# rubiruchi/ofdm_uhd

Hardware: AMD Instinct MI355X
Metric: OFDM symbols/sec (TX+loopback RX) @ N_fft=512; packet CRC pass rate (higher is better)
Workload: dtype f32; 1 GPU; N_fft=512, occ=200, QPSK, CP=128, synthetic AWGN channel (BASELINE configs[1]); payload_bytes=1026, symbols_per_packet=22, streams=1, iq_buffers=1, parallelism=independent streams, 1 per GPU

## Files before the change

ofdm_uhd_amd/csrc/engine_rx.inc:

```

template <typename T>
static int dev_excl_scan(ofdm_handle* h, const T* d_in, uint64_t n, T* d_out, T* d_total) {
  const uint64_t nb = (n + SCAN_BLOCK - 1) / SCAN_BLOCK;
  HIPCHK(h, h->rx.partial.ensure(sizeof(T) * std::max<uint64_t>(nb, 1)));
  T* part = h->rx.partial.as<T>();
  if (n == 0) {
    if (d_total) HIPCHK(h, hipMemsetAsync(d_total, 0, sizeof(T), h->stream));
    return OFDM_OK;
  }
  hipLaunchKernelGGL(HIP_KERNEL_NAME(k_scan_partials<T>), dim3((unsigned)nb), dim3(256), 0, h->stream, d_in, n, part);
  hipLaunchKernelGGL(HIP_KERNEL_NAME(k_scan_top<T>), dim3(1), dim3(256), 0, h->stream, part, nb, d_total);
  hipLaunchKernelGGL(HIP_KERNEL_NAME(k_scan_final<T>), dim3((unsigned)nb), dim3(256), 0, h->stream, d_in, n, part, d_out);
  HIPCHK(h, hipGetLastError());
  return OFDM_OK;
}

template <int N, bool TWL, bool TAPS, bool CSI = false>
static int launch_demod_t(ofdm_handle* h, const DemodParams& q, size_t shmem) {
  constexpr int T = N / 8, FPW = demod_fpw(N);
  if (shmem > 64 * 1024)
    HIPCHK(h, hipFuncSetAttribute(reinterpret_cast<const void*>(&k_rx_demod<N, TWL, TAPS, CSI>),
                                  hipFuncAttributeMaxDynamicSharedMemorySize, (int)shmem));
  hipLaunchKernelGGL(HIP_KERNEL_NAME(k_rx_demod<N, TWL, TAPS, CSI>), dim3((q.nframes + FPW - 1) / FPW), dim3(T * FPW), shmem,
                     h->stream, q);
  HIPCHK(h, hipGetLastError());
  return OFDM_OK;
}
template <int N, bool TWL>
static int launch_demod_v(ofdm_handle* h, const DemodParams& q, size_t shmem) {
  if (q.csi_eq) return launch_demod_t<N, TWL, true, true>(h, q, shmem);
  const bool instr = q.tap_mode != 0 || q.tap_sampler || q.tap_fft || q.tap_acq || q.tap_sink || q.tap_demapped || q.qual;
  return instr ? launch_demod_t<N, TWL, true>(h, q, shmem) : launch_demod_t<N, TWL, false>(h, q, shmem);
}

template <int N>
static int launch_demod(ofdm_handle* h, const DemodParams& q0) {
  DemodParams q = q0;
  constexpr int T = N / 8, WAVES = demod_fpw(N) * ((T + WAVE - 1) / WAVE);
  const bool grid = q.grid != nullptr;
  const bool csi = q.csi_eq != nullptr;
  auto bytes = [&](bool twl, bool sm) {
    return (size_t)demod_lds_bytes(N, twl, sm, q.occ, q.arity, q.nmap, q.nbits, q.shift, grid, csi);
  };
  constexpr int CU_WAVES = 4 * demod_waves_per_simd(N);
  auto wgs = [&](size_t b) { return std::max<size_t>(1, std::min<size_t>(std::max(1, CU_WAVES / WAVES), CU_LDS_BYTES / b)); };
  constexpr bool base_twl = !fft_onebuf(N);
  const size_t w0 = wgs(bytes(base_twl, false));
  bool twl = base_twl;
  if constexpr (fft_onebuf(N)) twl = wgs(bytes(true, false)) == w0 && bytes(true, false) <= CU_LDS_BYTES;
  q.smap_lds = (wgs(bytes(twl, true)) == w0 && bytes(twl, true) <= CU_LDS_BYTES) ? 1 : 0;
  if (const char* e = getenv("OFDM_DEMOD_LDS")) {
    const int v = atoi(e);
    if constexpr (fft_onebuf(N)) twl = (v & 1) != 0;
    q.smap_lds = (v >> 1) & 1;
  }
  const size_t shmem = bytes(twl, q.smap_lds != 0);
  if (shmem > CU_LDS_BYTES) FAIL(h, OFDM_E_INVAL, "configuration needs more than 160 KiB of LDS in k_rx_demod");
  if constexpr (fft_onebuf(N)) {
    return twl ? launch_demod_v<N, true>(h, q, shmem) : launch_demod_v<N, false>(h, q, shmem);
  } else {
    return launch_demod_v<N, true>(h, q, shmem);
  }
}

static int run_demod(ofdm_handle* h, const DemodParams& q) {
  switch (h->N) {
    case 64: return launch_demod<64>(h, q);
    case 128: return launch_demod<128>(h, q);
    case 256: return launch_demod<256>(h, q);
    case 512: return launch_demod<512>(h, q);
    case 1024: return launch_demod<1024>(h, q);
    case 2048: return launch_demod<2048>(h, q);
    default: return launch_demod<4096>(h, q);
  }
}

enum { CT_CAND = 0, CT_OVERFLOW = 1, CT_NLO = 2, CT_NHI = 3, CT_CHAIN = 4, CT_NPEAKS = 5, CT_NSYM = 6, CT_KEYTOT = 7,
       CT_DEFR = 8 , CT_RAWTOT = 13, CT_PIECES = 14, CT_STASH = 15, CT_RECS = 16, CT_COUNT = 17 };

static int sync_params(ofdm_handle* h, uint64_t nsamples, bool cap_full, SyncParams* out) {
  RxState& rx = h->rx;
  const int N = h->N, CP = h->CP, T = SYNC_TILE;
  const uint64_t ntiles = (nsamples + T - 1) / T;
  const int tiles_per_seg = 32 * ((N + CP + T - 1) / T);
  const uint64_t egrid = std::min<uint64_t>(ntiles, 256ull * 8ull), egrid_small = std::min<uint64_t>(ntiles, 256ull * 16ull);
  const uint64_t cand_cap = (cap_full ? nsamples + nsamples / 8 : nsamples / 16) + (egrid + 16) * SYNC_CHUNK_C + egrid_small * 2048ull;
  const uint64_t piece_cap = (cap_full ? nsamples / 2 + 1 : nsamples / 128) + (egrid + egrid_small + 16) * SYNC_CHUNK_P;
  HIPCHK(h, rx.y.ensure(nsamples * sizeof(c32)));
  HIPCHK(h, rx.tile_B.ensure(ntiles * sizeof(double)));
  HIPCHK(h, rx.tile_np.ensure(ntiles * sizeof(uint32_t)));
  HIPCHK(h, rx.tile_pieces.ensure(piece_cap * sizeof(SyncPiece)));
  HIPCHK(h, rx.tile_first.ensure(ntiles * sizeof(uint64_t)));
  HIPCHK(h, rx.avg_in.ensure(ntiles * sizeof(double)));
  HIPCHK(h, rx.cand_u.ensure(cand_cap * sizeof(float)));
  HIPCHK(h, rx.cand_P.ensure(cand_cap * sizeof(c32)));
  HIPCHK(h, rx.counters.ensure(CT_COUNT * sizeof(uint64_t)));
  HIPCHK(h, rx.counts.ensure(ntiles * sizeof(uint32_t)));
  HIPCHK(h, rx.offsets.ensure(ntiles * sizeof(uint32_t)));
  HIPCHK(h, rx.recs.ensure(ntiles * sizeof(SyncRec)));
  float *d_metric = nullptr, *d_presel = nullptr;
  if (h->tap_mask & (1u << OFDM_TAP_RX_METRIC)) {
    HIPCHK(h, rx.metric.ensure(nsamples * sizeof(float)));
    d_metric = rx.metric.as<float>();
  }
  if (h->tap_mask & (1u << OFDM_TAP_RX_PRESEL)) {
    HIPCHK(h, rx.presel.ensure(nsamples * sizeof(float)));
    d_presel = rx.presel.as<float>();
  }
  uint64_t* ctr = rx.counters.as<uint64_t>();
  SyncParams sp;
  memset(&sp, 0, sizeof(sp));
  sp.N = N;
  sp.D = N / 2;
  sp.CP = CP;
  sp.HY = (N + 7) / 8 * 8;
  sp.HM = CP;
  sp.R = sync_ring_samples(sp.HY);
  sp.tiles_per_seg = tiles_per_seg;
  sp.nsamples = nsamples;
  sp.ntiles = ntiles;
  sp.tapcp = (float)(1.0 / (double)CP);
  sp.cand_thr = -fmaxf(h->cfg.peak_rise, h->cfg.peak_fall);
  sp.alpha = h->cfg.peak_alpha;
  sp.decay = (double)(1.0f - h->cfg.peak_alpha);
  sp.y = rx.y.as<c32>();
  sp.metric_tap = d_metric;
  sp.presel_tap = d_presel;
  sp.dpow = h->d_synctab.as<double>();
  sp.ipow = sp.dpow + (SYNC_TILE + 1);
  sp.wtab = reinterpret_cast<const float*>(sp.ipow + (SYNC_TILE + 1));
  sp.tile_B = rx.tile_B.as<double>();
  sp.tile_npieces = rx.tile_np.as<uint32_t>();
  sp.tile_first = rx.tile_first.as<uint64_t>();
  sp.pieces = rx.tile_pieces.as<SyncPiece>();
  sp.piece_cap = piece_cap;
  sp.piece_count = reinterpret_cast<unsigned long long*>(ctr + CT_PIECES);
  sp.cand_u = rx.cand_u.as<float>();
  sp.cand_P = rx.cand_P.as<c32>();
  sp.cand_cap = cand_cap;
  sp.cand_count = reinterpret_cast<unsigned long long*>(ctr + CT_CAND);
  sp.overflow = reinterpret_cast<unsigned int*>(ctr + CT_OVERFLOW);
  sp.recs = rx.recs.as<SyncRec>();
  sp.rec_count = reinterpret_cast<unsigned long long*>(ctr + CT_RECS);
  sp.exact_small = sync_exact_small(CP, N / 2);
  if (const char* es = getenv("OFDM_EXACT_SMALL")) sp.exact_small = std::max(0, std::min(atoi(es), (int)SYNC_TILE));
#ifdef SYNC_DIAG
  if (const char* ab = getenv("OFDM_ABLATE")) sp.ablate = atoi(ab);
#endif
  if (sp.HM > T) FAIL(h, OFDM_E_INVAL, "cyclic prefix longer than a k_sync tile");
  *out = sp;
  return OFDM_OK;
}

static uint64_t sync_nseg(const SyncParams& sp) { return (sp.ntiles + (uint64_t)sp.tiles_per_seg - 1) / (uint64_t)sp.tiles_per_seg; }

#ifdef SYNC_STAMPS
static DevBuf g_stamp_buf;
static int stamps_prepare(ofdm_handle* h, SyncParams& sp, uint64_t nseg) {
  HIPCHK(h, g_stamp_buf.ensure(nseg * 16 * sizeof(unsigned long long)));
  HIPCHK(h, hipMemsetAsync(g_stamp_buf.p, 0, nseg * 16 * sizeof(unsigned long long), h->stream));
  sp.stamps = g_stamp_buf.as<unsigned long long>();
  return OFDM_OK;
}
static int sync_stamps_report(ofdm_handle* h, const unsigned long long* d_stamps, uint64_t nseg, int tiles_per_seg) {
  HIPCHK(h, hipStreamSynchronize(h->stream));
  std::vector<unsigned long long> st(nseg * 16);
  HIPCHK(h, hipMemcpy(st.data(), d_stamps, st.size() * 8, hipMemcpyDeviceToHost));
  double sum[16] = {0};
  for (uint64_t i = 0; i < nseg; i++)
    for (int k = 0; k < 16; k++) sum[k] += (double)st[i * 16 + k];
  const char* nm[16] = {"-", "y tile -> ring / filter", "B2 wait", "terms", "scan3 (B3)", "M + B4", "mavg + B5", "summary", "filter: block A", "filter: block B", "filter: taps + windows in", "-", "-", "-", "-", "-"};
  double tot = 0;
  for (int k = 0; k < 16; k++) tot += sum[k];
  fprintf(stderr, "[k_sync stamps] %llu workgroups, s_memtime ticks per workgroup-tile (wave 0):\n", (unsigned long long)nseg);
  for (int k = 0; k < 11; k++)
    fprintf(stderr, "  %-26s %10.0f  %5.1f%%\n", nm[k], sum[k] / (double)nseg / (double)(tiles_per_seg + 1), 100.0 * sum[k] / tot);
  return OFDM_OK;
}
#endif

static bool front_fused(const ofdm_handle* h) {
  if (h->cfg.sync_mode != OFDM_SYNC_PN) return false;
  const char* e = getenv("OFDM_FRONT");
  if (!e || atoi(e) == 0) return false;
  const int F = h->filtF, B = F - (int)h->cfg.ntaps + 1;
  if (F > 512) return false;
  const int HY = (h->N + 7) / 8 * 8, C = (B + 7) / 8 * 8;
  if (HY + C > SYNC_TILE || h->CP > SYNC_TILE) return false;
  return front_lds_layout(sync_ring_samples(HY), h->CP, B, F).total <= CU_LDS_BYTES / 3;
}

static int launch_sync(ofdm_handle* h, SyncParams& sp) {
  RxState& rx = h->rx;
  const int T = SYNC_TILE;
  const uint64_t nseg = sync_nseg(sp);
  HIPCHK(h, hipMemsetAsync(rx.counters.p, 0, CT_COUNT * sizeof(uint64_t), h->stream));
#ifdef SYNC_STAMPS
  if (int rs = stamps_prepare(h, sp, nseg)) return rs;
#endif
  const size_t sync_shmem = sync_lds_layout(sp.R, sp.HM).total;
  if (sync_shmem > CU_LDS_BYTES) FAIL(h, OFDM_E_INVAL, "configuration needs more than 160 KiB of LDS in k_sync");
  {
    ProfScope span(h->prof, OFDM_K_SYNC, h->stream);
    int wg = (int)std::min<size_t>(SYNC_MAX_WG, CU_LDS_BYTES / sync_shmem);
    if (const char* w = getenv("OFDM_SYNC_W")) wg = std::min(wg, atoi(w));
    bool fixed_layout = sp.R - (int)T <= (int)T;
    if (const char* e = getenv("OFDM_SYNC_STATIC")) fixed_layout = fixed_layout && atoi(e) != 0;
    const void* fn = fixed_layout ? (wg >= 6   ? reinterpret_cast<const void*>(&k_sync<6, true>)
                                     : wg == 5 ? reinterpret_cast<const void*>(&k_sync<5, true>)
                                     : wg == 4 ? reinterpret_cast<const void*>(&k_sync<4, true>)
                                     : wg == 3 ? reinterpret_cast<const void*>(&k_sync<3, true>)
                                               : reinterpret_cast<const void*>(&k_sync<2, true>))
                                  : (wg >= 4   ? reinterpret_cast<const void*>(&k_sync<4, false>)
                                     : wg == 3 ? reinterpret_cast<const void*>(&k_sync<3, false>)
                                               : reinterpret_cast<const void*>(&k_sync<2, false>));
    HIPCHK(h, hipFuncSetAttribute(fn, hipFuncAttributeMaxDynamicSharedMemorySize, (int)sync_shmem));
    FilterParams nofp;
    memset(&nofp, 0, sizeof(nofp));
    void* args[] = {&sp, &nofp};
    HIPCHK(h, hipLaunchKernel(fn, dim3((unsigned)nseg), dim3(SYNC_THREADS), args, sync_shmem, h->stream));
  }
  HIPCHK(h, hipGetLastError());
  return OFDM_OK;
}

static void rx_note_input(ofdm_handle* h, const ofdm_c32* iq, uint64_t nsamples) {
  std::swap(h->ev_rx_in, h->ev_rx_in_old);
  h->rx_in_old_pending = h->rx_in_pending;
  h->rx_in_lo[1] = h->rx_in_lo[0];
  h->rx_in_hi[1] = h->rx_in_hi[0];
  h->rx_in_lo[0] = (uintptr_t)iq;
  h->rx_in_hi[0] = (uintptr_t)iq + nsamples * rx_ss(h);
}

static int launch_front(ofdm_handle* h, FilterParams& fp, uint64_t nsamples) {
  const int F = h->filtF;
  SyncParams sp;
  int rcs = sync_params(h, nsamples, false, &sp);
  if (rcs != OFDM_OK) return rcs;
  HIPCHK(h, hipMemsetAsync(h->rx.counters.p, 0, CT_COUNT * sizeof(uint64_t), h->stream));
  const size_t shm = front_lds_layout(sp.R, sp.HM, fp.B, F).total;
  const uint64_t nseg = sync_nseg(sp);
  const void* fn = F == 64    ? reinterpret_cast<const void*>(&k_sync<3, true, 64>)
                   : F == 128 ? reinterpret_cast<const void*>(&k_sync<3, true, 128>)
                   : F == 256 ? reinterpret_cast<const void*>(&k_sync<3, true, 256>)
                              : reinterpret_cast<const void*>(&k_sync<3, true, 512>);
  HIPCHK(h, hipFuncSetAttribute(fn, hipFuncAttributeMaxDynamicSharedMemorySize, (int)shm));
#ifdef SYNC_STAMPS
  if (int rs = stamps_prepare(h, sp, nseg)) return rs;
#endif
  void* args[] = {&sp, &fp};
  {
    ProfScope span(h->prof, OFDM_K_FRONT, h->stream);
    HIPCHK(h, hipLaunchKernel(fn, dim3((unsigned)nseg), dim3(SYNC_THREADS), args, shm, h->stream));
  }
  HIPCHK(h, hipGetLastError());
#ifdef SYNC_STAMPS
  if (int rs = sync_stamps_report(h, sp.stamps, nseg, sp.tiles_per_seg)) return rs;
#endif
  h->rx.front_done = true;
  return OFDM_OK;
}

template <typename XT>
static int launch_filter_t(ofdm_handle* h, FilterParams& fp, uint64_t nsamples) {
  const int F = h->filtF;
  const uint64_t bpr = 256 / (F / 8);
  const uint64_t nblk = (nsamples + (uint64_t)fp.goff + (uint64_t)fp.B - 1) / (uint64_t)fp.B;
  fp.nrounds = (nblk + bpr - 1) / bpr;
  const size_t fsh = (size_t)256 * 9 * sizeof(c32);
  const unsigned fgrid = (unsigned)std::min<uint64_t>(fp.nrounds, 256ull * 8ull * 4ull);
  {
    ProfScope span(h->prof, OFDM_K_FILTER, h->stream);
    switch (F) {
      case 64: hipLaunchKernelGGL(HIP_KERNEL_NAME(k_chan_filter<64, XT>), dim3(fgrid), dim3(256), fsh, h->stream, fp); break;
      case 128: hipLaunchKernelGGL(HIP_KERNEL_NAME(k_chan_filter<128, XT>), dim3(fgrid), dim3(256), fsh, h->stream, fp); break;
      case 256: hipLaunchKernelGGL(HIP_KERNEL_NAME(k_chan_filter<256, XT>), dim3(fgrid), dim3(256), fsh, h->stream, fp); break;
      case 512: hipLaunchKernelGGL(HIP_KERNEL_NAME(k_chan_filter<512, XT>), dim3(fgrid), dim3(256), fsh, h->stream, fp); break;
      case 1024: hipLaunchKernelGGL(HIP_KERNEL_NAME(k_chan_filter<1024, XT>), dim3(fgrid), dim3(256), fsh, h->stream, fp); break;
      default: FAIL(h, OFDM_E_INVAL, "unsupported channel filter transform length");
    }
  }
  HIPCHK(h, hipGetLastError());
  return OFDM_OK;
}

static int launch_filter(ofdm_handle* h, FilterParams& fp, uint64_t nsamples) {
  return h->rx_fmt == OFDM_IQ_SC16 ? launch_filter_t<sc16>(h, fp, nsamples) : launch_filter_t<c32>(h, fp, nsamples);
}

static int rx_submit_impl(ofdm_handle* h, const ofdm_c32* iq, uint64_t nsamples, const c32** d_x_out) {
  RxState& rx = h->rx;
  HIPCHK(h, hipSetDevice(h->cfg.device_id));
  if (h->tx_pending && h->txs != h->stream) HIPCHK(h, hipStreamWaitEvent(h->stream, h->ev_tx_done, 0));
  h->tx_pending = false;
  const c32* d_x = reinterpret_cast<const c32*>(iq);
  if (h->rx_fmt == OFDM_IQ_SC16) {
    if ((uintptr_t)iq & 3u) FAIL(h, OFDM_E_INVAL, "ofdm_sc16 buffers must be 4-byte aligned");
    if (front_fused(h)) FAIL(h, OFDM_E_INVAL, "the fused front end (OFDM_FRONT=1) takes float32 samples only");
  }
  if (!h->dev_ptrs) {
    HIPCHK(h, rx.x_stage.ensure(nsamples * rx_ss(h)));
    HIPCHK(h, hipMemcpyAsync(rx.x_stage.p, iq, nsamples * rx_ss(h), hipMemcpyHostToDevice, h->stream));
    d_x = rx.x_stage.as<c32>();
  }
  *d_x_out = d_x;
  rx.in_event_at_end = true;
  if (h->cfg.sync_mode != OFDM_SYNC_PN) return OFDM_OK;
  HIPCHK(h, rx.y.ensure(nsamples * sizeof(c32)));
  FilterParams fp;
  memset(&fp, 0, sizeof(fp));
  fp.B = h->filtF - (int)h->cfg.ntaps + 1;
  fp.ntm1 = (int)h->cfg.ntaps - 1;
  fp.goff = (int)(rx.origin % (uint64_t)fp.B);
  fp.nsamples = nsamples;
  fp.x = d_x;
  fp.y = rx.y.as<c32>();
  fp.Hf = h->d_Hf.as<c32>();
  fp.twF = h->d_twF.as<c32>();
  fp.xscale = h->rx_scale;
  rx.front_done = false;
  if (int rc = front_fused(h) ? launch_front(h, fp, nsamples) : launch_filter(h, fp, nsamples)) return rc;
  if (!h->sense.rx_on) {
    rx_note_input(h, iq, nsamples);
    HIPCHK(h, hipEventRecord(h->ev_rx_in, h->stream));
    h->rx_in_pending = true;
    rx.in_event_at_end = false;
  }
  return OFDM_OK;
}

extern "C" int ofdm_rx_submit(ofdm_handle* h, const ofdm_c32* iq, uint64_t nsamples) {
  if (!h) return OFDM_E_INVAL;
  if (nsamples && !iq) FAIL(h, OFDM_E_INVAL, "null argument");
  RxState& rx = h->rx;
  rx.sub_valid = false;
  if (nsamples == 0) return OFDM_OK;
  const c32* d_x = nullptr;
  int rc = rx_submit_impl(h, iq, nsamples, &d_x);
  if (rc != OFDM_OK) return rc;
  rx.sub_valid = true;
  rx.sub_iq = iq;
  rx.sub_n = nsamples;
  rx.sub_dx = d_x;
  rx.sub_hold = rx.in_event_at_end;
  return OFDM_OK;
}

struct RxCall {
  ofdm_handle* h;
  const ofdm_c32* iq;
  uint64_t nsamples;
  uint8_t* payload_out;
  uint64_t payload_cap;
  uint64_t* payload_off;
  uint32_t* payload_len;
  uint8_t* crc_ok;
  int max_pkts;
  int* npkt;
  ofdm_stats* stats;
  const c32* d_x = nullptr;
  bool fixed = false;
  bool done = false;
  bool dyn = false;
  uint64_t npeaks = 0, nforced = 0;
  uint64_t n_lo = 0, nframes = 0, nsym = 0, npk = 0, nbytes = 0, rawtot = 0;
  uint64_t npk_ub = 0;
  DynFrames dynf;
  DemodParams dq;
  DeframeParams fq;
  CsiRows csi_fr = {nullptr, nullptr, nullptr, nullptr};
  uint8_t* d_pay = nullptr;
};

static uint64_t* rx_ctr(ofdm_handle* h) { return h->rx.counters.as<uint64_t>(); }

static int rx_read_counts(RxCall& c) {
  ofdm_handle* h = c.h;
  RxState& rx = h->rx;
  uint64_t hc[CT_COUNT];
  HIPCHK(h, hipMemcpyAsync(hc, rx.counters.p, sizeof(hc), hipMemcpyDeviceToHost, h->stream));
  HIPCHK(h, hipStreamSynchronize(h->stream));
  c.n_lo = hc[CT_NLO] & 0xFFFFFFFFull;
  c.nframes = c.npeaks - c.n_lo - (hc[CT_NHI] & 0xFFFFFFFFull);
  c.nsym = hc[CT_NSYM];
  c.npk = hc[CT_KEYTOT] >> 40;
  c.nbytes = hc[CT_KEYTOT] & ((1ull << 40) - 1);
  c.rawtot = hc[CT_RAWTOT];
  rx.nframes = c.nframes;
  rx.j0 = c.n_lo;
  rx.nsym_total = c.nsym;
  if (c.stats) {
    c.stats->frames = c.nframes;
    c.stats->symbols = c.nsym;
    c.stats->headers_ok = hc[CT_DEFR + 0];
    c.stats->chained_frames = hc[CT_DEFR + 3];
    c.stats->overflow = hc[CT_OVERFLOW] & 0xFFFFFFFFull;
  }
  return OFDM_OK;
}

static int rx_check_capacity(RxCall& c) {
  if (c.npk <= (uint64_t)c.max_pkts && c.nbytes <= c.payload_cap) return OFDM_OK;
  *c.npkt = (int)std::min<uint64_t>(c.npk, 0x7FFFFFFF);
  FAIL(c.h, OFDM_E_CAPACITY, "payload_out / max_pkts too small for the packets found");
}

static hipError_t launch_sync_exact(const void* fn, unsigned grid, size_t shmem, SyncParams sp, hipStream_t s) {
  void* args[] = {&sp};
  return hipLaunchKernel(fn, dim3(grid), dim3(SYNC_THREADS), args, shmem, s);
}

static int rx_sync_exact(RxCall& c, SyncParams& sp, bool cap_full) {
  ofdm_handle* h = c.h;
  if (cap_full) {
    int rcs = sync_params(h, c.nsamples, true, &sp);
    if (rcs != OFDM_OK) return rcs;
    uint64_t* ctr = rx_ctr(h);
    HIPCHK(h, hipMemsetAsync(ctr + CT_CAND, 0, 2 * sizeof(uint64_t), h->stream));
    HIPCHK(h, hipMemsetAsync(ctr + CT_NPEAKS, 0, sizeof(uint64_t), h->stream));
    HIPCHK(h, hipMemsetAsync(ctr + CT_PIECES, 0, 2 * sizeof(uint64_t), h->stream));
  }
  const unsigned egrid = (unsigned)std::min<uint64_t>(sp.ntiles, 256ull * 8ull);
  const unsigned egrid_small = (unsigned)std::min<uint64_t>(sp.ntiles, 256ull * 16ull);
  {
    ProfScope span(h->prof, OFDM_K_EXACT, h->stream);
    const size_t esh = exact_lds_layout(sp.CP, SYNC_TILE).total, esh_small = exact_lds_layout(sp.CP, sp.exact_small).total;
    const void* fbig = sp.D >= 2048 ? reinterpret_cast<const void*>(&k_sync_exact<SYNC_THREADS, true>)
                                    : reinterpret_cast<const void*>(&k_sync_exact<SYNC_THREADS, false>);
    if (esh > 64 * 1024) HIPCHK(h, hipFuncSetAttribute(fbig, hipFuncAttributeMaxDynamicSharedMemorySize, (int)esh));
    if (sp.exact_small > 0)
      hipLaunchKernelGGL(HIP_KERNEL_NAME(k_sync_exact<WAVE, false>), dim3(egrid_small), dim3(WAVE), esh_small, h->stream, sp);
    HIPCHK(h, launch_sync_exact(fbig, egrid, esh, sp, h->stream));
    if (sp.metric_tap) {
      SyncParams tp = sp;
      tp.tap_only = 1;
      HIPCHK(h, launch_sync_exact(fbig, egrid, esh, tp, h->stream));
    }
  }
  HIPCHK(h, hipGetLastError());
#ifdef SYNC_STAMPS
  if (!h->rx.front_done)
    if (int rs = sync_stamps_report(h, sp.stamps, sync_nseg(sp), sp.tiles_per_seg)) return rs;
#endif
  return OFDM_OK;
}

static int rx_sense_fork(RxCall& c) {
  ofdm_handle* h = c.h;
  SenseState& ss = h->sense;
  HIPCHK(h, hipEventRecord(ss.ev_in, h->stream));
  HIPCHK(h, hipStreamWaitEvent(ss.side, ss.ev_in, 0));
  int src = sense_enqueue(h, &ss.rx_cfg, c.d_x, c.nsamples, ss.side);
  if (src != OFDM_OK) return src;
  HIPCHK(h, hipEventRecord(ss.ev_out, ss.side));
  return OFDM_OK;
}

static PeakParams make_peak_params(ofdm_handle* h, const SyncParams& sp) {
  RxState& rx = h->rx;
  PeakParams pp;
  memset(&pp, 0, sizeof(pp));
  pp.ntiles = sp.ntiles;
  pp.nsamples = sp.nsamples;
  pp.rise = h->cfg.peak_rise;
  pp.fall = h->cfg.peak_fall;
  pp.alpha = h->cfg.peak_alpha;
  pp.dpow = sp.dpow;
  pp.tile_npieces = rx.tile_np.as<uint32_t>();
  pp.tile_first = rx.tile_first.as<uint64_t>();
  pp.pieces = rx.tile_pieces.as<SyncPiece>();
  pp.avg_in = rx.avg_in.as<double>();
  pp.cand_u = rx.cand_u.as<float>();
  pp.cand_P = rx.cand_P.as<c32>();
  pp.counts = rx.counts.as<uint32_t>();
  pp.offsets = rx.offsets.as<uint32_t>();
  pp.stash_peaks = rx.stash_peaks.as<uint64_t>();
  pp.stash_P = rx.stash_P.as<c32>();
  pp.stash_overflow = reinterpret_cast<unsigned int*>(rx_ctr(h) + CT_STASH);
  if (h->tap_mask & (1u << OFDM_TAP_RX_RUN_AVG)) pp.run_rows = rx.run_rows.as<double>();
  return pp;
}

static int rx_flags_pn(RxCall& c, const SyncParams& sp, uint64_t* overflow) {
  ofdm_handle* h = c.h;
  RxState& rx = h->rx;
  const uint64_t ntiles = sp.ntiles;
  const unsigned grid = (unsigned)((ntiles + 255) / 256);
  uint64_t* ctr = rx_ctr(h);
  const uint64_t run_cap = (h->tap_mask & (1u << OFDM_TAP_RX_RUN_AVG)) ? sp.piece_cap : 0;
  HIPCHK(h, rx.stash_peaks.ensure(ntiles * PEAK_STASH * sizeof(uint64_t)));
  HIPCHK(h, rx.stash_P.ensure(ntiles * PEAK_STASH * sizeof(c32)));
  if (run_cap) HIPCHK(h, rx.run_rows.ensure(run_cap * 2 * sizeof(double)));
  PeakParams pp = make_peak_params(h, sp);
  hipLaunchKernelGGL(k_avg_carry, dim3(grid), dim3(256), 0, h->stream, rx.tile_B.as<double>(), ntiles, c.nsamples, sp.dpow,
                     rx.avg_in.as<double>());
  if (run_cap) HIPCHK(h, hipMemsetAsync(rx.run_rows.p, 0xFF, run_cap * 2 * sizeof(double), h->stream));
  hipLaunchKernelGGL(HIP_KERNEL_NAME(k_peak<false>), dim3(grid), dim3(256), 0, h->stream, pp);
  HIPCHK(h, hipGetLastError());
  int rc = dev_excl_scan<uint32_t>(h, rx.counts.as<uint32_t>(), ntiles, rx.offsets.as<uint32_t>(),
                                   reinterpret_cast<uint32_t*>(ctr + CT_NPEAKS));
  if (rc) return rc;
  uint64_t hc[CT_COUNT];
  HIPCHK(h, hipMemcpyAsync(hc, ctr, sizeof(hc), hipMemcpyDeviceToHost, h->stream));
  HIPCHK(h, hipStreamSynchronize(h->stream));
  if ((*overflow = hc[CT_OVERFLOW] & 0xFFFFFFFFull)) return OFDM_OK;
  rx.run_slots = std::min<uint64_t>(hc[CT_PIECES], run_cap);
  const uint64_t npeaks = hc[CT_NPEAKS] & 0xFFFFFFFFull;
  c.npeaks = rx.npeaks = npeaks;
  if (c.stats) c.stats->peaks = npeaks;
  if (npeaks == 0 && !(rx.nco_ref_on && !rx.hist_flags.empty())) {
    c.done = true;
    return OFDM_OK;
  }
  HIPCHK(h, rx.peaks.ensure(std::max<uint64_t>(npeaks, 1) * sizeof(uint64_t)));
  HIPCHK(h, rx.peak_P.ensure(std::max<uint64_t>(npeaks, 1) * sizeof(c32)));
  pp.peaks = rx.peaks.as<uint64_t>();
  pp.peak_P = rx.peak_P.as<c32>();
  if (npeaks > 0) {
    if (hc[CT_STASH] & 0xFFFFFFFFull)
      hipLaunchKernelGGL(HIP_KERNEL_NAME(k_peak<true>), dim3(grid), dim3(256), 0, h->stream, pp);
    else
      hipLaunchKernelGGL(k_peak_compact, dim3(grid), dim3(256), 0, h->stream, pp);
    HIPCHK(h, hipGetLastError());
  }
  return OFDM_OK;
}

__global__ void __launch_bounds__(256) k_fixed_flags(uint64_t npeaks, uint64_t first, uint64_t period, uint64_t* __restrict__ peaks,
                                                      c32* __restrict__ peak_P) {
  const uint64_t k = (uint64_t)blockIdx.x * blockDim.x + threadIdx.x;
  if (k >= npeaks) return;
  peaks[k] = first + k * period;
  peak_P[k] = mk(0.f, 0.f);
}

static int rx_fixed_count(RxCall& c) {
  ofdm_handle* h = c.h;
  RxState& rx = h->rx;
  const uint64_t L = (uint64_t)h->L;
  c.npeaks = rx.npeaks = c.nsamples >= L ? (c.nsamples - L) / ((uint64_t)h->cfg.fixed_nsymbols * L) + 1 : 0;
  if (c.stats) c.stats->peaks = c.npeaks;
  HIPCHK(h, rx.counters.ensure(CT_COUNT * sizeof(uint64_t)));
  HIPCHK(h, hipMemsetAsync(rx.counters.p, 0, CT_COUNT * sizeof(uint64_t), h->stream));
  if (c.npeaks == 0) {
    HIPCHK(h, hipStreamSynchronize(h->stream));
    c.done = true;
  }
  return OFDM_OK;
}

static int rx_flags_fixed(RxCall& c) {
  ofdm_handle* h = c.h;
  RxState& rx = h->rx;
  HIPCHK(h, rx.peaks.ensure(c.npeaks * sizeof(uint64_t)));
  HIPCHK(h, rx.peak_P.ensure(c.npeaks * sizeof(c32)));
  hipLaunchKernelGGL(k_fixed_flags, dim3((unsigned)((c.npeaks + 255) / 256)), dim3(256), 0, h->stream, c.npeaks, (uint64_t)h->L - 1,
                     (uint64_t)h->cfg.fixed_nsymbols * (uint64_t)h->L, rx.peaks.as<uint64_t>(), rx.peak_P.as<c32>());
  HIPCHK(h, hipGetLastError());
  return OFDM_OK;
}

static int rx_splice(RxCall& c) {
  ofdm_handle* h = c.h;
  RxState& rx = h->rx;
  if (!rx.nco_ref_on) return OFDM_OK;
  const uint64_t npeaks = c.npeaks;
  std::vector<uint64_t> hp(npeaks);
  if (npeaks) HIPCHK(h, hipMemcpyAsync(hp.data(), rx.peaks.p, npeaks * sizeof(uint64_t), hipMemcpyDeviceToHost, h->stream));
  HIPCHK(h, hipStreamSynchronize(h->stream));
  uint64_t kdrop = 0;
  while (kdrop < npeaks && (int64_t)hp[kdrop] <= rx.nco_trust_after) kdrop++;
  const uint64_t m = rx.hist_flags.size(), np2 = m + npeaks - kdrop;
  c.done = np2 == 0;
  if (!c.done) {
    HIPCHK(h, rx.peaks2.ensure(np2 * sizeof(uint64_t)));
    HIPCHK(h, rx.peak_P2.ensure(np2 * sizeof(c32)));
    HIPCHK(h, rx.fstep.ensure(std::max<uint64_t>(m, 1) * sizeof(double)));
    if (m) {
      HIPCHK(h, hipMemcpyAsync(rx.peaks2.p, rx.hist_flags.data(), m * sizeof(uint64_t), hipMemcpyHostToDevice, h->stream));
      HIPCHK(h, hipMemsetAsync(rx.peak_P2.p, 0, m * sizeof(c32), h->stream));
      HIPCHK(h, hipMemcpyAsync(rx.fstep.p, rx.hist_steps.data(), m * sizeof(double), hipMemcpyHostToDevice, h->stream));
    }
    if (npeaks > kdrop) {
      HIPCHK(h, hipMemcpyAsync(rx.peaks2.as<uint64_t>() + m, rx.peaks.as<uint64_t>() + kdrop, (npeaks - kdrop) * sizeof(uint64_t),
                               hipMemcpyDeviceToDevice, h->stream));
      HIPCHK(h, hipMemcpyAsync(rx.peak_P2.as<c32>() + m, rx.peak_P.as<c32>() + kdrop, (npeaks - kdrop) * sizeof(c32),
                               hipMemcpyDeviceToDevice, h->stream));
    }
    HIPCHK(h, hipStreamSynchronize(h->stream));
    std::swap(rx.peaks, rx.peaks2);
    std::swap(rx.peak_P, rx.peak_P2);
    c.nforced = m;
  }
  c.npeaks = rx.npeaks = np2;
  if (c.stats) c.stats->peaks = np2;
  return OFDM_OK;
}

static FramesParams make_frames_params(const RxCall& c) {
  ofdm_handle* h = c.h;
  RxState& rx = h->rx;
  uint64_t* ctr = rx_ctr(h);
  FramesParams fp;
  memset(&fp, 0, sizeof(fp));
  fp.npeaks = c.npeaks;
  fp.nsamples = c.nsamples;
  fp.N = h->N;
  fp.L = h->L;
  fp.timeout = h->cfg.sampler_timeout;
  fp.sens = (float)(-2.0 / (double)h->N);
  fp.peaks = rx.peaks.as<uint64_t>();
  fp.peak_P = rx.peak_P.as<c32>();
  fp.angle = rx.angle.as<float>();
  fp.step = rx.step.as<double>();
  fp.inc = rx.inc.as<uint64_t>();
  fp.K = rx.K.as<uint32_t>();
  fp.nsym = rx.nsym.as<uint64_t>();
  fp.n_lo = reinterpret_cast<unsigned int*>(ctr + CT_NLO);
  fp.n_hi = reinterpret_cast<unsigned int*>(ctr + CT_NHI);
  fp.nforced = c.nforced;
  fp.forced_step = rx.fstep.as<double>();
  fp.fixed_on = c.fixed ? 1 : 0;
  fp.fixed_angle = h->cfg.fixed_freq_offset;
  return fp;
}

static int rx_frames(RxCall& c) {
  ofdm_handle* h = c.h;
  RxState& rx = h->rx;
  const uint64_t npeaks = c.npeaks;
  const unsigned grid = (unsigned)((npeaks + 255) / 256);
  HIPCHK(h, rx.angle.ensure(npeaks * sizeof(float)));
  HIPCHK(h, rx.step.ensure(npeaks * sizeof(double)));
  HIPCHK(h, rx.inc.ensure(npeaks * sizeof(uint64_t)));
  HIPCHK(h, rx.inc_acc.ensure(npeaks * sizeof(uint64_t)));
  HIPCHK(h, rx.Phi_u.ensure(npeaks * sizeof(uint64_t)));
  HIPCHK(h, rx.Phi.ensure(npeaks * sizeof(double)));
  HIPCHK(h, rx.K.ensure(npeaks * sizeof(uint32_t)));
  HIPCHK(h, rx.nsym.ensure(npeaks * sizeof(uint64_t)));
  HIPCHK(h, rx.sym_base.ensure(npeaks * sizeof(uint64_t)));
  const FramesParams fp = make_frames_params(c);
  const uint64_t ref_u = rx.nco_ref_on ? rx.nco_ref_u : 0ull;
  c.dq.ref_on = (rx.nco_ref_on || (c.fixed && h->cfg.fixed_freq_offset != 0.0f)) ? 1 : 0;
  c.dq.ref_peak = rx.nco_ref_on ? rx.nco_ref_peak : 0;
  c.dq.ref_phi = nco_radians(ref_u);
  c.dq.ref_step = rx.nco_ref_on ? rx.nco_ref_step : (double)(fp.sens * h->cfg.fixed_freq_offset);
  hipLaunchKernelGGL(k_frames, dim3(grid), dim3(256), 0, h->stream, fp);
  HIPCHK(h, hipGetLastError());
  int rc = dev_excl_scan<uint64_t>(h, rx.inc.as<uint64_t>(), npeaks, rx.inc_acc.as<uint64_t>(), (uint64_t*)nullptr);
  if (rc) return rc;
  hipLaunchKernelGGL(k_nco_phase, dim3(grid), dim3(256), 0, h->stream, rx.peaks.as<uint64_t>(), rx.inc_acc.as<uint64_t>(), npeaks,
                     c.dq.ref_on, c.dq.ref_peak, ref_u, c.dq.ref_step, rx.Phi_u.as<uint64_t>(), rx.Phi.as<double>());
  HIPCHK(h, hipGetLastError());
  return dev_excl_scan<uint64_t>(h, rx.nsym.as<uint64_t>(), npeaks, rx.sym_base.as<uint64_t>(), rx_ctr(h) + CT_NSYM);
}

static int rx_timing(RxCall& c) {
  ofdm_handle* h = c.h;
  SyncParams sp;
  uint64_t overflow = 0;
  int rc = c.fixed ? rx_fixed_count(c) : sync_params(h, c.nsamples, false, &sp);
  if (rc || c.done) return rc;
  if (!c.fixed && !h->rx.front_done && (rc = launch_sync(h, sp))) return rc;
  for (int attempt = 0; attempt < 2; attempt++) {
    if (!c.fixed && (rc = rx_sync_exact(c, sp, attempt == 1))) return rc;
    if (!c.fixed && attempt == 0 && h->sense.rx_on && (rc = rx_sense_fork(c))) return rc;
    ProfScope span(h->prof, OFDM_K_PEAK, h->stream);
    if ((rc = c.fixed ? rx_flags_fixed(c) : rx_flags_pn(c, sp, &overflow))) return rc;
    if (overflow) continue;
    if (c.done) {
      span.end();
      HIPCHK(h, hipStreamSynchronize(h->stream));
      return OFDM_OK;
    }
    if ((rc = rx_splice(c)) || c.done) return rc;
    return rx_frames(c);
  }
  if (c.stats) c.stats->overflow = overflow;
  FAIL(h, OFDM_E_OVERFLOW, "candidate / piece buffer exhausted");
}

static size_t csi_bytes(uint64_t rows, uint64_t stride) { return rows * stride * (sizeof(c32) + 3 * sizeof(float)); }
static CsiRows csi_carve(const DevBuf& b, uint64_t rows, uint64_t stride) {
  const uint64_t cell = rows * stride;
  CsiRows r;
  r.eq = b.as<c32>();
  r.pre = reinterpret_cast<float*>(r.eq + cell);
  r.err = r.pre + cell;
  r.ref = r.err + cell;
  return r;
}

static int make_demod_params(RxCall& c) {
  ofdm_handle* h = c.h;
  RxState& rx = h->rx;
  DemodParams& dq = c.dq;
  dq.dyn = c.dynf;
  dq.N = h->N;
  dq.CP = h->CP;
  dq.L = h->L;
  dq.occ = h->occ;
  dq.zl = h->zl;
  dq.nmap = h->nmap;
  dq.nbits = h->nbits;
  dq.arity = (int)h->cfg.arity;
  dq.shift = (int)h->cfg.max_fft_shift_len;
  dq.phase_gain = h->cfg.phase_gain;
  dq.freq_gain = h->cfg.freq_gain;
  dq.eq_gain = h->cfg.eq_gain;
  dq.sign_kind = h->sign_kind;
  memcpy(dq.sign_idx, h->sign_idx, 4);
  dq.sign_eps = h->sign_eps;
  dq.sign_bound = h->sign_bound;
  dq.nsamples = c.nsamples;
  dq.j0 = (uint32_t)c.n_lo;
  dq.nframes = (uint32_t)c.nframes;
  dq.npeaks = (uint32_t)c.npeaks;
  dq.y = rx.y_ptr;
  dq.peaks = rx.peaks.as<uint64_t>();
  dq.Phi = rx.Phi.as<double>();
  dq.step = rx.step.as<double>();
  dq.K = rx.K.as<uint32_t>();
  dq.sym_base = rx.sym_base.as<uint64_t>();
  dq.tw = h->d_tw.as<c32>();
  dq.ks = h->d_ks.as<c32>();
  dq.kd = h->d_kd.as<float>();
  dq.smap = h->d_smap.as<int16_t>();
  dq.constellation = h->d_const.as<c32>();
  dq.grid = h->has_grid ? h->d_grid.as<SlicerGrid>() : nullptr;
  dq.invalid = rx.invalid.as<uint8_t>();
  dq.res = rx.res.as<FrameResult>();
  dq.raw = rx.raw.as<uint8_t>();
  if (rx.quality_on) {
    HIPCHK(h, rx.qual_frame.ensure(c.nframes * sizeof(FrameQuality)));
    dq.qual = rx.qual_frame.as<FrameQuality>();
  }
  if (rx.csi_on) {
    rx.csi_stride = (h->occ + 3) & ~3;
    HIPCHK(h, rx.csi_frame.ensure(csi_bytes(c.nframes, (uint64_t)rx.csi_stride)));
    c.csi_fr = csi_carve(rx.csi_frame, c.nframes, (uint64_t)rx.csi_stride);
    dq.csi_eq = c.csi_fr.eq;
    dq.csi_pre = c.csi_fr.pre;
    dq.csi_err = c.csi_fr.err;
    dq.csi_ref = c.csi_fr.ref;
    dq.csi_stride = rx.csi_stride;
  }
  return OFDM_OK;
}

#ifdef SYNC_STAMPS
static int demod_stamps_report(ofdm_handle* h) {
  HIPCHK(h, hipStreamSynchronize(h->stream));
  unsigned long long st[16];
  HIPCHK(h, hipMemcpyFromSymbol(st, HIP_SYMBOL(g_demod_stamps), sizeof(st)));
  const unsigned long long zero[16] = {0};
  HIPCHK(h, hipMemcpyToSymbol(HIP_SYMBOL(g_demod_stamps), zero, sizeof(zero)));
  const char* nm[8] = {"frame prologue", "derotation (+ sample wait)", "transform", "prefetch issue + spectrum to LDS", "frame acquisition",
                       "demapper", "loop bookkeeping", "PLL, header, bytes"};
  double tot = 0;
  for (int k = 0; k < 8; k++) tot += (double)st[k];
  fprintf(stderr, "[k_rx_demod stamps] s_memtime ticks summed over the workgroups' thread 0 (%.3e in all):\n", tot);
  for (int k = 0; k < 8; k++) fprintf(stderr, "  %-34s %12.4e  %5.1f%%\n", nm[k], (double)st[k], 100.0 * (double)st[k] / (tot > 0 ? tot : 1));
  return OFDM_OK;
}
#endif

static int rx_demodulate(RxCall& c) {
  ofdm_handle* h = c.h;
  RxState& rx = h->rx;
  const uint64_t nframes = c.nframes;
  HIPCHK(h, rx.res.ensure(nframes * sizeof(FrameResult)));
  HIPCHK(h, rx.raw.ensure(nframes * (uint64_t)RAW_SLOT));
  HIPCHK(h, rx.invalid.ensure(nframes));
  HIPCHK(h, rx.chain_list.ensure(4096 * sizeof(uint32_t)));
  HIPCHK(h, rx.key.ensure(nframes * sizeof(uint64_t)));
  HIPCHK(h, rx.pos.ensure(nframes * sizeof(uint64_t)));
  HIPCHK(h, hipMemsetAsync(rx.invalid.p, 0, nframes, h->stream));
  int rc = make_demod_params(c);
  if (rc) return rc;
  ProfScope span(h->prof, OFDM_K_DEMOD, h->stream);
  rc = run_demod(h, c.dq);
#ifdef SYNC_STAMPS
  if (rc == OFDM_OK) rc = demod_stamps_report(h);
#endif
  return rc;
}

static int rx_chains(RxCall& c) {
  ofdm_handle* h = c.h;
  RxState& rx = h->rx;
  uint64_t* ctr = rx_ctr(h);
  const uint32_t nframes = (uint32_t)c.nframes;
  hipLaunchKernelGGL(k_chain_collect, dim3((nframes + 255) / 256), dim3(256), 0, h->stream, rx.res.as<FrameResult>(), nframes, c.dynf,
                     rx.chain_list.as<uint32_t>(), 4096u, reinterpret_cast<unsigned int*>(ctr + CT_CHAIN));
  uint32_t npre = 0;
  std::vector<uint8_t> pre_host;
  if (rx.nco_ref_on && c.nforced > c.n_lo) {
    npre = (uint32_t)std::min<uint64_t>(c.nforced - c.n_lo, c.nframes);
    pre_host.assign(rx.hist_swallowed.begin() + c.n_lo, rx.hist_swallowed.begin() + c.n_lo + npre);
    HIPCHK(h, rx.pre_inv.ensure(npre));
    HIPCHK(h, hipMemcpyAsync(rx.pre_inv.p, pre_host.data(), npre, hipMemcpyHostToDevice, h->stream));
  }
  hipLaunchKernelGGL(k_chain_resolve, dim3(1), dim3(64), 0, h->stream, rx.res.as<FrameResult>(), nframes, c.dynf,
                     rx.chain_list.as<uint32_t>(), 4096u, reinterpret_cast<const unsigned int*>(ctr + CT_CHAIN),
                     rx.invalid.as<uint8_t>(), reinterpret_cast<unsigned int*>(ctr + CT_OVERFLOW), rx.pre_inv.as<uint8_t>(), npre);
  HIPCHK(h, hipGetLastError());
  if (npre) HIPCHK(h, hipStreamSynchronize(h->stream));
  return OFDM_OK;
}

static int rx_tap_pass(RxCall& c) {
  ofdm_handle* h = c.h;
  RxState& rx = h->rx;
  const uint32_t tapm = h->tap_mask;
  auto on = [&](int tap) { return (tapm >> tap) & 1u; };
  const uint64_t nsamples = c.nsamples, nsym = c.nsym;
  if (on(OFDM_TAP_RX_SIGMIX) || on(OFDM_TAP_RX_NCO)) {
    c32 *d_sm = nullptr, *d_nco = nullptr;
    if (on(OFDM_TAP_RX_SIGMIX)) {
      HIPCHK(h, rx.tap_sigmix.ensure(nsamples * sizeof(c32)));
      d_sm = rx.tap_sigmix.as<c32>();
    }
    if (on(OFDM_TAP_RX_NCO)) {
      HIPCHK(h, rx.tap_nco.ensure(nsamples * sizeof(c32)));
      d_nco = rx.tap_nco.as<c32>();
    }
    hipLaunchKernelGGL(k_sigmix_tap, dim3((unsigned)((nsamples + 255) / 256)), dim3(256), 0, h->stream, rx.y_ptr, nsamples,
                       rx.peaks.as<uint64_t>(), rx.Phi.as<double>(), rx.step.as<double>(), c.npeaks, c.dq.ref_on, c.dq.ref_peak,
                       c.dq.ref_phi, c.dq.ref_step, d_sm, d_nco);
    HIPCHK(h, hipGetLastError());
  }
  if (!(on(OFDM_TAP_RX_FFT) || on(OFDM_TAP_RX_ACQ) || on(OFDM_TAP_RX_SINK) || on(OFDM_TAP_RX_SAMPLER))) return OFDM_OK;
  DemodParams tq = c.dq;
  tq.tap_mode = 1;
  tq.qual = nullptr;
  tq.csi_eq = nullptr;
  tq.csi_pre = tq.csi_err = tq.csi_ref = nullptr;
  if (on(OFDM_TAP_RX_SAMPLER)) {
    HIPCHK(h, rx.tap_sampler.ensure(nsym * (uint64_t)h->N * sizeof(c32)));
    tq.tap_sampler = rx.tap_sampler.as<c32>();
  }
  if (on(OFDM_TAP_RX_FFT)) {
    HIPCHK(h, rx.tap_fft.ensure(nsym * (uint64_t)h->N * sizeof(c32)));
    tq.tap_fft = rx.tap_fft.as<c32>();
  }
  if (on(OFDM_TAP_RX_ACQ)) {
    HIPCHK(h, rx.tap_acq.ensure(nsym * (uint64_t)h->occ * sizeof(c32)));
    tq.tap_acq = rx.tap_acq.as<c32>();
  }
  if (on(OFDM_TAP_RX_SINK)) {
    HIPCHK(h, rx.tap_sink.ensure(nsym * (uint64_t)h->occ * sizeof(c32)));
    HIPCHK(h, rx.tap_demapped.ensure(nsym));
    HIPCHK(h, hipMemsetAsync(rx.tap_sink.p, 0, nsym * (uint64_t)h->occ * sizeof(c32), h->stream));
    HIPCHK(h, hipMemsetAsync(rx.tap_demapped.p, 0, nsym, h->stream));
    tq.tap_sink = rx.tap_sink.as<c32>();
    tq.tap_demapped = rx.tap_demapped.as<uint8_t>();
  }
  return run_demod(h, tq);
}

static DeframeParams make_deframe_params(const RxCall& c) {
  ofdm_handle* h = c.h;
  RxState& rx = h->rx;
  DeframeParams fq;
  memset(&fq, 0, sizeof(fq));
  fq.dyn = c.dynf;
  fq.nframes = (uint32_t)c.nframes;
  fq.res = rx.res.as<FrameResult>();
  fq.invalid = rx.invalid.as<uint8_t>();
  fq.raw = rx.raw.as<uint8_t>();
  fq.mask = h->d_mask.as<uint8_t>();
  fq.crc_table = h->d_crc.as<uint32_t>();
  fq.xp8 = h->d_xp8.as<uint32_t>();
  fq.key = rx.key.as<uint64_t>();
  fq.pos = rx.pos.as<uint64_t>();
  fq.counters = rx_ctr(h) + CT_DEFR;
  return fq;
}

static int rx_deframe_count(RxCall& c) {
  ofdm_handle* h = c.h;
  RxState& rx = h->rx;
  const uint64_t nframes = c.nframes;
  const unsigned grid = (unsigned)((nframes + 255) / 256);
  c.fq = make_deframe_params(c);
  hipLaunchKernelGGL(k_deframe_count, dim3(grid), dim3(256), 0, h->stream, c.fq);
  HIPCHK(h, hipGetLastError());
  int rc = dev_excl_scan<uint64_t>(h, rx.key.as<uint64_t>(), nframes, rx.pos.as<uint64_t>(), rx_ctr(h) + CT_KEYTOT);
  if (rc) return rc;
  if (h->tap_mask & (1u << OFDM_TAP_RX_PACKETS)) {
    HIPCHK(h, rx.raw_lens.ensure(nframes * sizeof(uint64_t)));
    HIPCHK(h, rx.raw_pos.ensure(nframes * sizeof(uint64_t)));
    hipLaunchKernelGGL(k_raw_len, dim3(grid), dim3(256), 0, h->stream, c.fq, rx.raw_lens.as<uint64_t>());
    rc = dev_excl_scan<uint64_t>(h, rx.raw_lens.as<uint64_t>(), nframes, rx.raw_pos.as<uint64_t>(), rx_ctr(h) + CT_RAWTOT);
  }
  return rc;
}

static QualityParams make_quality_params(ofdm_handle* h) {
  RxState& rx = h->rx;
  QualityParams qw;
  qw.fq = rx.qual_frame.as<FrameQuality>();
  qw.step = rx.step.as<double>();
  qw.out = rx.qual_out.as<ofdm_pkt_quality>();
  qw.inv_npilot = h->q_npilot ? 1.0f / (float)h->q_npilot : 0.0f;
  qw.inv_nnull = h->q_nnull ? 1.0f / (float)h->q_nnull : 0.0f;
  qw.N = h->N;
  qw.nmap = h->nmap;
  return qw;
}

static int rx_outputs(RxCall& c) {
  ofdm_handle* h = c.h;
  RxState& rx = h->rx;
  DeframeParams& fq = c.fq;
  const uint64_t nframes = c.nframes;
  const uint64_t npk_ub = c.npk_ub = c.dyn ? std::min<uint64_t>(nframes, (uint64_t)c.max_pkts) : c.npk;
  c.d_pay = c.payload_out;
  if (npk_ub == 0) return OFDM_OK;
  HIPCHK(h, rx.out_off.ensure((npk_ub + 1) * sizeof(uint64_t)));
  HIPCHK(h, rx.out_len.ensure(npk_ub * sizeof(uint32_t)));
  HIPCHK(h, rx.out_ok.ensure(npk_ub));
  HIPCHK(h, rx.out_pos.ensure(npk_ub * sizeof(uint64_t)));
  if (!h->dev_ptrs) {
    const uint64_t stage = c.dyn ? std::min<uint64_t>(c.payload_cap, nframes * (uint64_t)OFDM_MAX_PKT_LEN) : c.nbytes;
    HIPCHK(h, rx.out_payload.ensure(std::max<uint64_t>(stage, 1)));
    c.d_pay = rx.out_payload.as<uint8_t>();
  }
  fq.payload_out = c.d_pay;
  fq.payload_cap = c.dyn ? c.payload_cap : c.nbytes;
  fq.out_off = rx.out_off.as<uint64_t>();
  fq.out_len = rx.out_len.as<uint32_t>();
  fq.out_ok = rx.out_ok.as<uint8_t>();
  fq.out_pos = rx.out_pos.as<uint64_t>();
  fq.peaks = rx.peaks.as<uint64_t>();
  fq.j0 = (uint32_t)c.n_lo;
  fq.max_pkts = (uint32_t)npk_ub;
  hipLaunchKernelGGL(k_deframe_write, dim3((unsigned)((nframes + 3) / 4)), dim3(256), 0, h->stream, fq);
  HIPCHK(h, hipGetLastError());
  if (rx.quality_on) {
    HIPCHK(h, rx.qual_out.ensure(npk_ub * sizeof(ofdm_pkt_quality)));
    hipLaunchKernelGGL(k_quality_write, dim3((unsigned)((nframes + 255) / 256)), dim3(256), 0, h->stream, fq, make_quality_params(h));
    HIPCHK(h, hipGetLastError());
  }
  if (rx.csi_on) {
    HIPCHK(h, rx.csi_rows.ensure(csi_bytes(npk_ub, (uint64_t)rx.csi_stride)));
    rx.csi_rows_cap = npk_ub;
    hipLaunchKernelGGL(k_csi_write, dim3((unsigned)((nframes + 3) / 4)), dim3(256), 0, h->stream, fq, c.csi_fr,
                       csi_carve(rx.csi_rows, npk_ub, (uint64_t)rx.csi_stride), rx.csi_stride);
    HIPCHK(h, hipGetLastError());
  }
  if (h->tap_mask & (1u << OFDM_TAP_RX_PACKETS)) {
    rx.raw_tap_bytes = c.rawtot;
    HIPCHK(h, rx.raw_tap.ensure(std::max<uint64_t>(rx.raw_tap_bytes, 1)));
    hipLaunchKernelGGL(k_raw_tap, dim3((unsigned)((nframes + 255) / 256)), dim3(256), 0, h->stream, fq, rx.raw_pos.as<uint64_t>(),
                       rx.raw_tap.as<uint8_t>());
    HIPCHK(h, hipGetLastError());
  }
  HIPCHK(h, hipMemcpyAsync(c.payload_off, rx.out_off.p, npk_ub * sizeof(uint64_t), hipMemcpyDeviceToHost, h->stream));
  HIPCHK(h, hipMemcpyAsync(c.payload_len, rx.out_len.p, npk_ub * sizeof(uint32_t), hipMemcpyDeviceToHost, h->stream));
  HIPCHK(h, hipMemcpyAsync(c.crc_ok, rx.out_ok.p, npk_ub, hipMemcpyDeviceToHost, h->stream));
  rx.last_pos.resize(npk_ub);
  HIPCHK(h, hipMemcpyAsync(rx.last_pos.data(), rx.out_pos.p, npk_ub * sizeof(uint64_t), hipMemcpyDeviceToHost, h->stream));
  if (rx.quality_on) {
    rx.last_quality.resize(npk_ub);
    HIPCHK(h, hipMemcpyAsync(rx.last_quality.data(), rx.qual_out.p, npk_ub * sizeof(ofdm_pkt_quality), hipMemcpyDeviceToHost,
                             h->stream));
  }
  if (!c.dyn && !h->dev_ptrs && c.nbytes)
    HIPCHK(h, hipMemcpyAsync(c.payload_out, c.d_pay, c.nbytes, hipMemcpyDeviceToHost, h->stream));
  return OFDM_OK;
}

static int rx_finish(RxCall& c) {
  ofdm_handle* h = c.h;
  RxState& rx = h->rx;
  int rc = rx_read_counts(c);
  if (rc) return rc;
  const uint64_t npk = c.npk, nframes = c.nframes;
  if (c.dyn) {
    rx.last_pos.resize(std::min<uint64_t>(npk, c.npk_ub));
    if (rx.quality_on) rx.last_quality.resize(std::min<uint64_t>(npk, c.npk_ub));
    if ((rc = rx_check_capacity(c))) return rc;
    if (!h->dev_ptrs && c.nbytes) HIPCHK(h, hipMemcpy(c.payload_out, c.d_pay, c.nbytes, hipMemcpyDeviceToHost));
  }
  rx.last_swallowed.assign(rx.npeaks, 0);
  if (nframes) {
    std::vector<uint8_t> inv(nframes);
    HIPCHK(h, hipMemcpy(inv.data(), rx.invalid.p, nframes, hipMemcpyDeviceToHost));
    for (uint64_t f = 0; f < nframes && rx.j0 + f < rx.npeaks; f++) rx.last_swallowed[rx.j0 + f] = inv[f];
  }
  if (npk > 0) c.payload_off[npk] = c.nbytes;
  *c.npkt = (int)npk;
  if (rx.csi_on) {
    rx.csi_n = npk;
    rx.csi_ok.assign(c.crc_ok, c.crc_ok + npk);
  }
  if (c.stats) {
    uint64_t nok = 0;
    for (uint64_t i = 0; i < npk; i++) nok += c.crc_ok[i] ? 1 : 0;
    c.stats->packets = npk;
    c.stats->crc_ok = nok;
  }
  return OFDM_OK;
}

static int rx_begin(RxCall& c) {
  ofdm_handle* h = c.h;
  if (!c.npkt || c.max_pkts < 0 || (c.nsamples && !c.iq)) FAIL(h, OFDM_E_INVAL, "null argument");
  if (c.max_pkts > 0 && (!c.payload_off || !c.payload_len || !c.crc_ok)) FAIL(h, OFDM_E_INVAL, "null metadata array");
  *c.npkt = 0;
  if (c.payload_off) c.payload_off[0] = 0;
  if (c.stats) memset(c.stats, 0, sizeof(*c.stats));
  RxState& rx = h->rx;
  rx.nsamples = c.nsamples;
  rx.npeaks = rx.nframes = rx.j0 = rx.nsym_total = rx.raw_tap_bytes = rx.run_slots = 0;
  rx.last_pos.clear();
  rx.last_swallowed.clear();
  rx.last_quality.clear();
  rx.quality_valid = rx.quality_on;
  rx.csi_valid = rx.csi_on;
  rx.csi_n = 0;
  rx.csi_ok.clear();
  if (c.stats) c.stats->samples = c.nsamples;
  return OFDM_OK;
}

static int rx_input(RxCall& c) {
  ofdm_handle* h = c.h;
  RxState& rx = h->rx;
  if (rx.sub_valid && rx.sub_iq == c.iq && rx.sub_n == c.nsamples) {
    c.d_x = rx.sub_dx;
    rx.in_event_at_end = h->cfg.sync_mode != OFDM_SYNC_PN || h->sense.rx_on;
  } else {
    int rcs = rx_submit_impl(h, c.iq, c.nsamples, &c.d_x);
    if (rcs != OFDM_OK) return rcs;
  }
  rx.sub_valid = false;
  rx.y_ptr = c.fixed ? c.d_x : rx.y.as<c32>();
  if (c.fixed && h->rx_fmt == OFDM_IQ_SC16) {
    HIPCHK(h, rx.y.ensure(c.nsamples * sizeof(c32)));
    const unsigned grid = (unsigned)std::min<uint64_t>((c.nsamples + 255) / 256, 256 * 8);
    hipLaunchKernelGGL(k_expand_sc16, dim3(grid), dim3(256), 0, h->stream, reinterpret_cast<const sc16*>(c.d_x), c.nsamples,
                       h->rx_scale, rx.y.as<c32>());
    HIPCHK(h, hipGetLastError());
    rx.y_ptr = rx.y.as<c32>();
  }
  return OFDM_OK;
}

static bool rx_counts_on_device(const ofdm_handle* h) {
  const uint32_t probes = (1u << OFDM_TAP_RX_SIGMIX) | (1u << OFDM_TAP_RX_NCO) | (1u << OFDM_TAP_RX_FFT) | (1u << OFDM_TAP_RX_ACQ) |
                          (1u << OFDM_TAP_RX_SINK) | (1u << OFDM_TAP_RX_SAMPLER) | (1u << OFDM_TAP_RX_PACKETS);
  return !h->rx.nco_ref_on && !(h->tap_mask & probes) && !getenv("OFDM_RX_SYNCS");
}

static int rx_impl(RxCall& c) {
  ofdm_handle* h = c.h;
  int rc = rx_begin(c);
  if (rc || c.nsamples == 0) return rc;
  HIPCHK(h, hipSetDevice(h->cfg.device_id));
  c.fixed = h->cfg.sync_mode == OFDM_SYNC_FIXED;
  if ((rc = rx_input(c))) return rc;
  if ((rc = rx_timing(c)) || c.done) return rc;
  c.dyn = rx_counts_on_device(h);
  c.nframes = c.npeaks;
  if (!c.dyn && ((rc = rx_read_counts(c)) || c.nframes == 0)) return rc;
  c.dynf.lo = c.dyn ? reinterpret_cast<const unsigned int*>(rx_ctr(h) + CT_NLO) : nullptr;
  c.dynf.hi = c.dyn ? reinterpret_cast<const unsigned int*>(rx_ctr(h) + CT_NHI) : nullptr;
  c.dynf.npeaks = (uint32_t)c.npeaks;
  if ((rc = rx_demodulate(c))) return rc;
  {
    ProfScope span(h->prof, OFDM_K_DEFRAME, h->stream);
    if ((rc = rx_chains(c)) || (rc = rx_tap_pass(c)) || (rc = rx_deframe_count(c))) return rc;
    if (!c.dyn && ((rc = rx_read_counts(c)) || (rc = rx_check_capacity(c)))) return rc;
    if ((rc = rx_outputs(c))) return rc;
  }
  return rx_finish(c);
}

extern "C" int ofdm_rx(ofdm_handle* h, const ofdm_c32* iq, uint64_t nsamples, uint8_t* payload_out, uint64_t payload_cap,
                       uint64_t* payload_off, uint32_t* payload_len, uint8_t* crc_ok, int max_pkts, int* npkt,
                       ofdm_stats* stats) {
  if (!h) return OFDM_E_INVAL;
  h->rx.in_event_at_end = false;
  RxCall c{h, iq, nsamples, payload_out, payload_cap, payload_off, payload_len, crc_ok, max_pkts, npkt, stats};
  const int rc = rx_impl(c);
  h->rx.sub_valid = false;
  h->rx.sub_hold = false;
  if (h->sense.rx_on && h->sense.side) (void)hipStreamSynchronize(h->sense.side);
  h->prof.collect();
  if (h->rx.in_event_at_end) {
    h->rx.in_event_at_end = false;
    rx_note_input(h, iq, nsamples);
    if (hipEventRecord(h->ev_rx_in, h->stream) == hipSuccess) h->rx_in_pending = true;
  }
  return rc;
}

static int copy_tap(ofdm_handle* h, const void* d_src, uint64_t bytes, void* out, uint64_t cap, uint64_t* nbytes) {
  if (nbytes) *nbytes = bytes;
  if (!out || bytes == 0) return OFDM_OK;
  if (cap < bytes) FAIL(h, OFDM_E_CAPACITY, "tap buffer too small");
  HIPCHK(h, hipMemcpy(out, d_src, bytes, hipMemcpyDeviceToHost));
  return OFDM_OK;
}

__global__ void k_gather_frames(const uint64_t* __restrict__ peaks, const uint32_t* __restrict__ K, uint64_t j0, uint64_t nframes,
                                uint64_t* __restrict__ out) {
  const uint64_t f = (uint64_t)blockIdx.x * blockDim.x + threadIdx.x;
  if (f >= nframes) return;
  out[2 * f] = peaks[j0 + f];
  out[2 * f + 1] = K[j0 + f];
}

extern "C" int ofdm_tap(ofdm_handle* h, int tap, void* out, uint64_t cap, uint64_t* nbytes) {
  if (!h) return OFDM_E_INVAL;
  if (tap < 0 || tap >= OFDM_TAP_COUNT) FAIL(h, OFDM_E_INVAL, "unknown tap");
  HIPCHK(h, hipSetDevice(h->cfg.device_id));
  HIPCHK(h, hipStreamSynchronize(h->stream));
  if (h->txs != h->stream) HIPCHK(h, hipStreamSynchronize(h->txs));
  RxState& rx = h->rx;
  const bool en = (h->tap_mask >> tap) & 1u;
  switch (tap) {
    case OFDM_TAP_TX_PACKETS:
      return copy_tap(h, h->d_framed.p, h->last_tx_framed_bytes, out, cap, nbytes);
    case OFDM_TAP_TX_FREQ:
      if (!en && !((h->tap_mask >> OFDM_TAP_TX_MAPPER) & 1u)) FAIL(h, OFDM_E_INVAL, "tap not enabled (ofdm_set_taps)");
      return copy_tap(h, h->d_freq_tap.p, h->last_tx_nsym * (uint64_t)h->N * sizeof(c32), out, cap, nbytes);
    case OFDM_TAP_RX_CHAN_FILT:
      return copy_tap(h, rx.y_ptr, rx.y_ptr ? rx.nsamples * sizeof(c32) : 0, out, cap, nbytes);
    case OFDM_TAP_TX_IFFT:
      if (!en) FAIL(h, OFDM_E_INVAL, "tap not enabled (ofdm_set_taps)");
      return copy_tap(h, h->d_ifft_tap.p, h->last_tx_nsym * (uint64_t)h->N * sizeof(c32), out, cap, nbytes);
    case OFDM_TAP_TX_MAPPER: {
      if (!en) FAIL(h, OFDM_E_INVAL, "tap not enabled (ofdm_set_taps)");
      const uint64_t rowb = (uint64_t)h->N * sizeof(c32);
      const uint64_t npk = h->last_sym_off.empty() ? 0 : h->last_sym_off.size() - 1;
      const uint64_t rows = h->last_tx_nsym - npk;
      if (nbytes) *nbytes = rows * rowb;
      if (!out || rows == 0) return OFDM_OK;
      if (cap < rows * rowb) FAIL(h, OFDM_E_CAPACITY, "tap buffer too small");
      uint64_t r = 0;
      for (uint64_t k = 0; k < npk; k++) {
        const uint64_t s0 = h->last_sym_off[k] + 1, s1 = h->last_sym_off[k + 1];
        if (s1 > s0)
          HIPCHK(h, hipMemcpy((uint8_t*)out + r * rowb, (const uint8_t*)h->d_freq_tap.p + s0 * rowb, (s1 - s0) * rowb, hipMemcpyDeviceToHost));
        r += s1 - s0;
      }
      return OFDM_OK;
    }
    case OFDM_TAP_RX_SAMPLER:
      if (!en) FAIL(h, OFDM_E_INVAL, "tap not enabled (ofdm_set_taps)");
      return copy_tap(h, rx.tap_sampler.p, rx.nframes ? rx.nsym_total * (uint64_t)h->N * sizeof(c32) : 0, out, cap, nbytes);
    case OFDM_TAP_RX_SIGMIX:
      if (!en) FAIL(h, OFDM_E_INVAL, "tap not enabled (ofdm_set_taps)");
      return copy_tap(h, rx.tap_sigmix.p, rx.nframes ? rx.nsamples * sizeof(c32) : 0, out, cap, nbytes);
    case OFDM_TAP_RX_NCO:
      if (!en) FAIL(h, OFDM_E_INVAL, "tap not enabled (ofdm_set_taps)");
      return copy_tap(h, rx.tap_nco.p, rx.nframes ? rx.nsamples * sizeof(c32) : 0, out, cap, nbytes);
    case OFDM_TAP_RX_METRIC:
      if (!en) FAIL(h, OFDM_E_INVAL, "tap not enabled (ofdm_set_taps)");
      if (h->cfg.sync_mode == OFDM_SYNC_FIXED) FAIL(h, OFDM_E_INVAL, "SYNC \"fixed\" computes no timing metric");
      return copy_tap(h, rx.metric.p, rx.nsamples * sizeof(float), out, cap, nbytes);
    case OFDM_TAP_RX_PRESEL:
      if (!en) FAIL(h, OFDM_E_INVAL, "tap not enabled (ofdm_set_taps)");
      if (h->cfg.sync_mode == OFDM_SYNC_FIXED) FAIL(h, OFDM_E_INVAL, "SYNC \"fixed\" computes no timing metric");
      return copy_tap(h, rx.presel.p, rx.nsamples * sizeof(float), out, cap, nbytes);
    case OFDM_TAP_RX_RUN_AVG: {
      if (!en) FAIL(h, OFDM_E_INVAL, "tap not enabled (ofdm_set_taps)");
      if (h->cfg.sync_mode == OFDM_SYNC_FIXED) FAIL(h, OFDM_E_INVAL, "SYNC \"fixed\" runs no peak detector");
      std::vector<double> all(rx.run_slots * 2);
      if (rx.run_slots) HIPCHK(h, hipMemcpy(all.data(), rx.run_rows.p, all.size() * sizeof(double), hipMemcpyDeviceToHost));
      std::vector<std::pair<double, double>> rows;
      for (uint64_t i = 0; i < rx.run_slots; i++)
        if (all[2 * i] == all[2 * i]) rows.emplace_back(all[2 * i], all[2 * i + 1]);
      std::sort(rows.begin(), rows.end());
      const uint64_t nb = rows.size() * 2 * sizeof(double);
      if (nbytes) *nbytes = nb;
      if (!out || nb == 0) return OFDM_OK;
      if (cap < nb) FAIL(h, OFDM_E_CAPACITY, "tap buffer too small");
      double* o = static_cast<double*>(out);
      for (size_t i = 0; i < rows.size(); i++) {
        o[2 * i] = rows[i].first;
        o[2 * i + 1] = rows[i].second;
      }
      return OFDM_OK;
    }
    case OFDM_TAP_RX_PEAKS:
      return copy_tap(h, rx.peaks.p, rx.npeaks * sizeof(uint64_t), out, cap, nbytes);
    case OFDM_TAP_RX_ANGLES:
      return copy_tap(h, rx.angle.p, rx.npeaks * sizeof(float), out, cap, nbytes);
    case OFDM_TAP_RX_FRAMES: {
      if (nbytes) *nbytes = rx.nframes * 2 * sizeof(uint64_t);
      if (!out || rx.nframes == 0) return OFDM_OK;
      HIPCHK(h, rx.partial.ensure(rx.nframes * 2 * sizeof(uint64_t)));
      hipLaunchKernelGGL(k_gather_frames, dim3((unsigned)((rx.nframes + 255) / 256)), dim3(256), 0, h->stream,
                         rx.peaks.as<uint64_t>(), rx.K.as<uint32_t>(), rx.j0, rx.nframes, rx.partial.as<uint64_t>());
      HIPCHK(h, hipStreamSynchronize(h->stream));
      return copy_tap(h, rx.partial.p, rx.nframes * 2 * sizeof(uint64_t), out, cap, nbytes);
    }
    case OFDM_TAP_RX_FFT:
      if (!en) FAIL(h, OFDM_E_INVAL, "tap not enabled (ofdm_set_taps)");
      return copy_tap(h, rx.tap_fft.p, rx.nframes ? rx.nsym_total * (uint64_t)h->N * sizeof(c32) : 0, out, cap, nbytes);
    case OFDM_TAP_RX_ACQ:
      if (!en) FAIL(h, OFDM_E_INVAL, "tap not enabled (ofdm_set_taps)");
      return copy_tap(h, rx.tap_acq.p, rx.nframes ? rx.nsym_total * (uint64_t)h->occ * sizeof(c32) : 0, out, cap, nbytes);
    case OFDM_TAP_RX_SINK: {
      if (!en) FAIL(h, OFDM_E_INVAL, "tap not enabled (ofdm_set_taps)");
      if (rx.nframes == 0 || rx.nsym_total == 0) {
        if (nbytes) *nbytes = 0;
        return OFDM_OK;
      }
      std::vector<uint8_t> flags(rx.nsym_total);
      HIPCHK(h, hipMemcpy(flags.data(), rx.tap_demapped.p, rx.nsym_total, hipMemcpyDeviceToHost));
      uint64_t rows = 0;
      for (uint64_t i = 0; i < rx.nsym_total; i++) rows += flags[i] ? 1 : 0;
      const uint64_t rowb = (uint64_t)h->occ * sizeof(c32);
      if (nbytes) *nbytes = rows * rowb;
      if (!out) return OFDM_OK;
      if (cap < rows * rowb) FAIL(h, OFDM_E_CAPACITY, "tap buffer too small");
      uint64_t r = 0;
      for (uint64_t i = 0; i < rx.nsym_total; i++)
        if (flags[i]) {
          HIPCHK(h, hipMemcpy((uint8_t*)out + r * rowb, (const uint8_t*)rx.tap_sink.p + i * rowb, rowb, hipMemcpyDeviceToHost));
          r++;
        }
      return OFDM_OK;
    }
    case OFDM_TAP_RX_PACKETS:
      if (!en) FAIL(h, OFDM_E_INVAL, "tap not enabled (ofdm_set_taps)");
      return copy_tap(h, rx.raw_tap.p, rx.raw_tap_bytes, out, cap, nbytes);
    case OFDM_TAP_RX_DEMAPPED:
      if (!((h->tap_mask >> OFDM_TAP_RX_SINK) & 1u)) FAIL(h, OFDM_E_INVAL, "tap needs OFDM_TAP_RX_SINK enabled (ofdm_set_taps)");
      return copy_tap(h, rx.tap_demapped.p, rx.nframes ? rx.nsym_total : 0, out, cap, nbytes);
  }
  return OFDM_E_INVAL;
}

extern "C" int ofdm_rx_packet_pos(ofdm_handle* h, uint64_t* pos, int cap, int* n) {
  if (!h) return OFDM_E_INVAL;
  const size_t np = h->rx.last_pos.size();
  if (n) *n = (int)np;
  if (np == 0 || !pos) return OFDM_OK;
  if ((size_t)cap < np) FAIL(h, OFDM_E_CAPACITY, "position array too small");
  memcpy(pos, h->rx.last_pos.data(), np * sizeof(uint64_t));
  return OFDM_OK;
}

extern "C" int ofdm_rx_nco_state(ofdm_handle* h, uint64_t* peaks, uint64_t* phi, double* step, uint8_t* swallowed, int cap,
                                 int* n) {
  if (!h) return OFDM_E_INVAL;
  RxState& rx = h->rx;
  if (n) *n = (int)std::min<uint64_t>(rx.npeaks, 0x7FFFFFFF);
  if (rx.npeaks == 0 || (!peaks && !phi && !step && !swallowed)) return OFDM_OK;
  if (!peaks || !phi || !step || !swallowed || (uint64_t)cap < rx.npeaks) FAIL(h, OFDM_E_CAPACITY, "NCO state arrays too small");
  for (uint64_t i = 0; i < rx.npeaks; i++) swallowed[i] = i < rx.last_swallowed.size() ? rx.last_swallowed[i] : 0;
  HIPCHK(h, hipSetDevice(h->cfg.device_id));
  HIPCHK(h, hipMemcpy(peaks, rx.peaks.p, rx.npeaks * sizeof(uint64_t), hipMemcpyDeviceToHost));
  HIPCHK(h, hipMemcpy(phi, rx.Phi_u.p, rx.npeaks * sizeof(uint64_t), hipMemcpyDeviceToHost));
  HIPCHK(h, hipMemcpy(step, rx.step.p, rx.npeaks * sizeof(double), hipMemcpyDeviceToHost));
  return OFDM_OK;
}

extern "C" int ofdm_rx_snr(const ofdm_handle* h, float* snr_est) {
  if (!h || !snr_est) return OFDM_E_INVAL;
  *snr_est = 0.0f;
  return OFDM_OK;
}

extern "C" int ofdm_set_rx_quality(ofdm_handle* h, int enable) {
  if (!h) return OFDM_E_INVAL;
  h->rx.quality_on = enable != 0;
  return OFDM_OK;
}

extern "C" int ofdm_rx_quality(ofdm_handle* h, ofdm_pkt_quality* out, int cap, int* n) {
  if (!h) return OFDM_E_INVAL;
  const RxState& rx = h->rx;
  if (!rx.quality_valid) FAIL(h, OFDM_E_INVAL, "the last ofdm_rx ran without link quality (ofdm_set_rx_quality)");
  const size_t np = rx.last_quality.size();
  if (n) *n = (int)np;
  if (np == 0 || !out) return OFDM_OK;
  if ((size_t)cap < np) FAIL(h, OFDM_E_CAPACITY, "quality array too small");
  memcpy(out, rx.last_quality.data(), np * sizeof(ofdm_pkt_quality));
  return OFDM_OK;
}

extern "C" int ofdm_set_rx_csi(ofdm_handle* h, int enable) {
  if (!h) return OFDM_E_INVAL;
  h->rx.csi_on = enable != 0;
  return OFDM_OK;
}

static CsiRows csi_packet_rows(const RxState& rx) { return csi_carve(rx.csi_rows, rx.csi_rows_cap, (uint64_t)rx.csi_stride); }

extern "C" int ofdm_rx_csi(ofdm_handle* h, int first, int count, ofdm_c32* eq, float* pre_power, float* err, float* ref, int* n) {
  if (!h) return OFDM_E_INVAL;
  if (!n) FAIL(h, OFDM_E_INVAL, "null argument");
  const RxState& rx = h->rx;
  if (!rx.csi_valid) FAIL(h, OFDM_E_INVAL, "the last ofdm_rx ran without channel state (ofdm_set_rx_csi)");
  *n = (int)rx.csi_n;
  if (count == 0) return OFDM_OK;
  if (first < 0 || count < 0 || (uint64_t)first + (uint64_t)count > rx.csi_n) FAIL(h, OFDM_E_INVAL, "rows out of range");
  HIPCHK(h, hipSetDevice(h->cfg.device_id));
  const CsiRows pk = csi_packet_rows(rx);
  const size_t st = (size_t)rx.csi_stride, occ = (size_t)h->occ, r0 = (size_t)first * st;
  if (eq)
    HIPCHK(h, hipMemcpy2DAsync(eq, occ * sizeof(c32), pk.eq + r0, st * sizeof(c32), occ * sizeof(c32), (size_t)count,
                               hipMemcpyDeviceToHost, h->stream));
  float* dst[3] = {pre_power, err, ref};
  const float* src[3] = {pk.pre, pk.err, pk.ref};
  for (int a = 0; a < 3; a++)
    if (dst[a])
      HIPCHK(h, hipMemcpy2DAsync(dst[a], occ * sizeof(float), src[a] + r0, st * sizeof(float), occ * sizeof(float), (size_t)count,
                                 hipMemcpyDeviceToHost, h->stream));
  HIPCHK(h, hipStreamSynchronize(h->stream));
  return OFDM_OK;
}

extern "C" int ofdm_rx_csi_summary(ofdm_handle* h, int crc_ok_only, uint32_t* npkt, double* pre_power, double* err, double* ref,
                                   double* inv_gain, uint32_t* ninv) {
  if (!h) return OFDM_E_INVAL;
  RxState& rx = h->rx;
  if (!rx.csi_valid) FAIL(h, OFDM_E_INVAL, "the last ofdm_rx ran without channel state (ofdm_set_rx_csi)");
  const int occ = h->occ;
  uint64_t np = 0;
  for (uint64_t p = 0; p < rx.csi_n; p++) np += (!crc_ok_only || rx.csi_ok[p]) ? 1 : 0;
  if (npkt) *npkt = (uint32_t)np;
  double* dst[CSI_S_COUNT] = {pre_power, err, ref, inv_gain};
  if (np == 0) {
    for (int k = 0; k < CSI_S_COUNT; k++)
      if (dst[k]) std::fill(dst[k], dst[k] + occ, 0.0);
    if (ninv) std::fill(ninv, ninv + occ, 0u);
    return OFDM_OK;
  }
  HIPCHK(h, hipSetDevice(h->cfg.device_id));
  CsiSumParams s;
  s.rows = csi_packet_rows(rx);
  s.ok = rx.out_ok.as<uint8_t>();
  s.npk = (uint32_t)rx.csi_n;
  s.occ = occ;
  s.stride = rx.csi_stride;
  s.crc_ok_only = crc_ok_only ? 1 : 0;
  s.nchunks = (uint32_t)((rx.csi_n + CSI_SUM_CHUNK - 1) / CSI_SUM_CHUNK);
  const uint64_t part = (uint64_t)s.nchunks * (uint64_t)occ;
  HIPCHK(h, rx.csi_part.ensure(part * (CSI_S_COUNT * sizeof(double) + sizeof(uint32_t))));
  HIPCHK(h, rx.csi_sum.ensure((uint64_t)occ * (CSI_S_COUNT * sizeof(double) + sizeof(uint32_t))));
  s.part = rx.csi_part.as<double>();
  s.part_n = reinterpret_cast<uint32_t*>(s.part + CSI_S_COUNT * part);
  s.out = rx.csi_sum.as<double>();
  s.out_n = reinterpret_cast<uint32_t*>(s.out + CSI_S_COUNT * occ);
  const unsigned gx = (unsigned)((occ + 255) / 256);
  hipLaunchKernelGGL(k_csi_summary, dim3(gx, s.nchunks), dim3(256), 0, h->stream, s);
  HIPCHK(h, hipGetLastError());
  hipLaunchKernelGGL(k_csi_summary_combine, dim3(gx), dim3(256), 0, h->stream, s);
  HIPCHK(h, hipGetLastError());
  for (int k = 0; k < CSI_S_COUNT; k++)
    if (dst[k])
      HIPCHK(h, hipMemcpyAsync(dst[k], s.out + (size_t)k * occ, occ * sizeof(double), hipMemcpyDeviceToHost, h->stream));
  if (ninv) HIPCHK(h, hipMemcpyAsync(ninv, s.out_n, occ * sizeof(uint32_t), hipMemcpyDeviceToHost, h->stream));
  HIPCHK(h, hipStreamSynchronize(h->stream));
  return OFDM_OK;
}

extern "C" int ofdm_rx_set_origin(ofdm_handle* h, uint64_t first_sample_index) {
  if (!h) return OFDM_E_INVAL;
  h->rx.origin = first_sample_index;
  return OFDM_OK;
}

extern "C" int ofdm_rx_set_flag_history(ofdm_handle* h, int enable, int n, const int64_t* flags, const double* steps,
                                        const uint8_t* swallowed, int64_t trust_after, int64_t pred_flag, uint64_t pred_phase, double pred_step) {
  if (!h) return OFDM_E_INVAL;
  RxState& rx = h->rx;
  rx.nco_ref_on = false;
  rx.hist_flags.clear();
  rx.hist_steps.clear();
  rx.hist_swallowed.clear();
  if (!enable) return OFDM_OK;
  if (n < 0 || (n > 0 && (!flags || !steps || !swallowed))) FAIL(h, OFDM_E_INVAL, "null argument");
  for (int i = 0; i < n; i++) {
    if (flags[i] < 0 || flags[i] > trust_after || (i > 0 && flags[i] <= flags[i - 1]) || flags[i] <= pred_flag)
      FAIL(h, OFDM_E_INVAL, "history flags must ascend inside [0, trust_after] and follow the predecessor");
    rx.hist_flags.push_back((uint64_t)flags[i]);
    rx.hist_steps.push_back(steps[i]);
    rx.hist_swallowed.push_back(swallowed[i]);
  }
  rx.nco_ref_on = true;
  rx.nco_trust_after = trust_after;
  rx.nco_ref_peak = pred_flag;
  rx.nco_ref_u = pred_phase;
  rx.nco_ref_step = pred_step;
  return OFDM_OK;
}
```

ofdm_uhd_amd/csrc/rx_state.h:

```cpp
#pragma once
#include "host_util.h"
#include "rx_demod.h"

#define RX_DEVBUFS(X)                                                                                                       \
  X(recs) X(x_stage) X(y) X(metric) X(presel) X(tile_B) X(tile_np) X(tile_first) X(tile_pieces) X(avg_in) X(cand_u)        \
  X(cand_P) X(counters) X(counts) X(offsets) X(partial) X(peaks) X(peak_P) X(angle) X(step) X(inc) X(Phi) X(K) X(nsym)     \
  X(sym_base) X(res) X(raw) X(invalid) X(chain_list) X(key) X(pos) X(out_payload) X(out_off) X(out_len) X(out_ok)          \
  X(out_pos) X(inc_acc) X(Phi_u) X(peaks2) X(peak_P2) X(fstep) X(pre_inv) X(stash_peaks) X(stash_P) X(tap_fft) X(tap_acq)  \
  X(tap_sink) X(tap_demapped) X(raw_tap) X(raw_lens) X(raw_pos) X(tap_sampler) X(tap_sigmix) X(tap_nco) X(qual_frame)      \
  X(qual_out) X(csi_frame) X(csi_rows) X(csi_part) X(csi_sum) X(run_rows)

struct RxState {
#define X(name) DevBuf name;
  RX_DEVBUFS(X)
#undef X
  uint64_t nsamples = 0, npeaks = 0, nframes = 0, j0 = 0, nsym_total = 0, raw_tap_bytes = 0;
  uint64_t run_slots = 0;
  const c32* y_ptr = nullptr;
  bool sub_valid = false, in_event_at_end = false;
  bool front_done = false;
  bool sub_hold = false;
  const void* sub_iq = nullptr;
  uint64_t sub_n = 0;
  const c32* sub_dx = nullptr;
  uint64_t origin = 0;
  std::vector<uint64_t> last_pos;
  bool nco_ref_on = false;
  int64_t nco_ref_peak = 0, nco_trust_after = 0;
  uint64_t nco_ref_u = 0;
  double nco_ref_step = 0.0;
  std::vector<uint64_t> hist_flags;
  std::vector<double> hist_steps;
  std::vector<uint8_t> hist_swallowed;
  std::vector<uint8_t> last_swallowed;
  bool quality_on = false, quality_valid = false;
  std::vector<ofdm_pkt_quality> last_quality;
  bool csi_on = false, csi_valid = false;
  uint64_t csi_n = 0, csi_rows_cap = 0;
  int csi_stride = 0;
  std::vector<uint8_t> csi_ok;
  void release() {
#define X(name) name.release();
    RX_DEVBUFS(X)
#undef X
  }
};
```

Before: 132.3 million OFDM symbols/s.

## Consolidate RX readback buffers into one pinned device-to-host block transfer

Packs counters, invalid flags, packet offsets, lengths, CRC flags, positions and quality records into a single device buffer with a fixed section layout. The end of RX then needs one device-to-host copy into a pinned host mirror. This replaces several separate async copies plus a synchronous pageable hipMemcpy of the invalid array. Host-side results become views into the pinned mirror rather than owned vectors, so their lifetime now depends on when the mirror is reallocated or views are dropped. Growing the block costs an extra device-to-device copy and a stream sync.

```diff
diff --git a/ofdm_uhd_amd/csrc/engine_rx.inc b/ofdm_uhd_amd/csrc/engine_rx.inc
--- a/ofdm_uhd_amd/csrc/engine_rx.inc
+++ b/ofdm_uhd_amd/csrc/engine_rx.inc
@@ -75,8 +75,40 @@
   }
 }
 
-enum { CT_CAND = 0, CT_OVERFLOW = 1, CT_NLO = 2, CT_NHI = 3, CT_CHAIN = 4, CT_NPEAKS = 5, CT_NSYM = 6, CT_KEYTOT = 7,
-       CT_DEFR = 8 , CT_RAWTOT = 13, CT_PIECES = 14, CT_STASH = 15, CT_RECS = 16, CT_COUNT = 17 };
+static uint64_t* rx_ctr(ofdm_handle* h) { return h->rx.rb.as<uint64_t>(); }
+
+static int rx_block_counters(ofdm_handle* h) {
+  HIPCHK(h, h->rx.rb.ensure(rx_readback_layout(0, 0, false).total));
+  return OFDM_OK;
+}
+
+static int rx_block_fit(ofdm_handle* h, const RxReadback& lay) {
+  RxState& rx = h->rx;
+  if (lay.total > rx.rb.cap) {
+    DevBuf nb;
+    HIPCHK(h, nb.ensure(lay.total));
+    hipError_t e = hipMemcpyAsync(nb.p, rx.rb.p, lay.s[RB_COUNTERS].bytes, hipMemcpyDeviceToDevice, h->stream);
+    if (e == hipSuccess) e = hipStreamSynchronize(h->stream);
+    if (e != hipSuccess) {
+      nb.release();
+      HIPCHK(h, e);
+    }
+    rx.rb.release();
+    rx.rb = nb;
+  }
+  rx.rb_lay = lay;
+  return OFDM_OK;
+}
+
+static int rx_fetch(ofdm_handle* h, size_t bytes, const uint64_t** counters) {
+  RxState& rx = h->rx;
+  if (bytes > rx.rb_host.cap) rx.drop_views();
+  HIPCHK(h, rx.rb_host.ensure(bytes));
+  HIPCHK(h, hipMemcpyAsync(rx.rb_host.p, rx.rb.p, bytes, hipMemcpyDeviceToHost, h->stream));
+  HIPCHK(h, hipStreamSynchronize(h->stream));
+  *counters = rx.rb_host.as<uint64_t>();
+  return OFDM_OK;
+}
 
 static int sync_params(ofdm_handle* h, uint64_t nsamples, bool cap_full, SyncParams* out) {
   RxState& rx = h->rx;
@@ -94,7 +126,7 @@
   HIPCHK(h, rx.avg_in.ensure(ntiles * sizeof(double)));
   HIPCHK(h, rx.cand_u.ensure(cand_cap * sizeof(float)));
   HIPCHK(h, rx.cand_P.ensure(cand_cap * sizeof(c32)));
-  HIPCHK(h, rx.counters.ensure(CT_COUNT * sizeof(uint64_t)));
+  if (int rcb = rx_block_counters(h)) return rcb;
   HIPCHK(h, rx.counts.ensure(ntiles * sizeof(uint32_t)));
   HIPCHK(h, rx.offsets.ensure(ntiles * sizeof(uint32_t)));
   HIPCHK(h, rx.recs.ensure(ntiles * sizeof(SyncRec)));
@@ -107,7 +139,7 @@
     HIPCHK(h, rx.presel.ensure(nsamples * sizeof(float)));
     d_presel = rx.presel.as<float>();
   }
-  uint64_t* ctr = rx.counters.as<uint64_t>();
+  uint64_t* ctr = rx_ctr(h);
   SyncParams sp;
   memset(&sp, 0, sizeof(sp));
   sp.N = N;
@@ -191,10 +223,9 @@
 }
 
 static int launch_sync(ofdm_handle* h, SyncParams& sp) {
-  RxState& rx = h->rx;
   const int T = SYNC_TILE;
   const uint64_t nseg = sync_nseg(sp);
-  HIPCHK(h, hipMemsetAsync(rx.counters.p, 0, CT_COUNT * sizeof(uint64_t), h->stream));
+  HIPCHK(h, hipMemsetAsync(rx_ctr(h), 0, CT_COUNT * sizeof(uint64_t), h->stream));
 #ifdef SYNC_STAMPS
   if (int rs = stamps_prepare(h, sp, nseg)) return rs;
 #endif
@@ -238,7 +269,7 @@
   SyncParams sp;
   int rcs = sync_params(h, nsamples, false, &sp);
   if (rcs != OFDM_OK) return rcs;
-  HIPCHK(h, hipMemsetAsync(h->rx.counters.p, 0, CT_COUNT * sizeof(uint64_t), h->stream));
+  HIPCHK(h, hipMemsetAsync(rx_ctr(h), 0, CT_COUNT * sizeof(uint64_t), h->stream));
   const size_t shm = front_lds_layout(sp.R, sp.HM, fp.B, F).total;
   const uint64_t nseg = sync_nseg(sp);
   const void* fn = F == 64    ? reinterpret_cast<const void*>(&k_sync<3, true, 64>)
@@ -373,14 +404,11 @@
   uint8_t* d_pay = nullptr;
 };
 
-static uint64_t* rx_ctr(ofdm_handle* h) { return h->rx.counters.as<uint64_t>(); }
-
-static int rx_read_counts(RxCall& c) {
-  ofdm_handle* h = c.h;
-  RxState& rx = h->rx;
-  uint64_t hc[CT_COUNT];
-  HIPCHK(h, hipMemcpyAsync(hc, rx.counters.p, sizeof(hc), hipMemcpyDeviceToHost, h->stream));
-  HIPCHK(h, hipStreamSynchronize(h->stream));
+static int rx_read_counts(RxCall& c, size_t bytes) {
+  ofdm_handle* h = c.h;
+  RxState& rx = h->rx;
+  const uint64_t* hc = nullptr;
+  if (int rcf = rx_fetch(h, bytes, &hc)) return rcf;
   c.n_lo = hc[CT_NLO] & 0xFFFFFFFFull;
   c.nframes = c.npeaks - c.n_lo - (hc[CT_NHI] & 0xFFFFFFFFull);
   c.nsym = hc[CT_NSYM];
@@ -501,9 +529,8 @@
   int rc = dev_excl_scan<uint32_t>(h, rx.counts.as<uint32_t>(), ntiles, rx.offsets.as<uint32_t>(),
                                    reinterpret_cast<uint32_t*>(ctr + CT_NPEAKS));
   if (rc) return rc;
-  uint64_t hc[CT_COUNT];
-  HIPCHK(h, hipMemcpyAsync(hc, ctr, sizeof(hc), hipMemcpyDeviceToHost, h->stream));
-  HIPCHK(h, hipStreamSynchronize(h->stream));
+  const uint64_t* hc = nullptr;
+  if ((rc = rx_fetch(h, CT_COUNT * sizeof(uint64_t), &hc))) return rc;
   if ((*overflow = hc[CT_OVERFLOW] & 0xFFFFFFFFull)) return OFDM_OK;
   rx.run_slots = std::min<uint64_t>(hc[CT_PIECES], run_cap);
   const uint64_t npeaks = hc[CT_NPEAKS] & 0xFFFFFFFFull;
@@ -541,8 +568,8 @@
   const uint64_t L = (uint64_t)h->L;
   c.npeaks = rx.npeaks = c.nsamples >= L ? (c.nsamples - L) / ((uint64_t)h->cfg.fixed_nsymbols * L) + 1 : 0;
   if (c.stats) c.stats->peaks = c.npeaks;
-  HIPCHK(h, rx.counters.ensure(CT_COUNT * sizeof(uint64_t)));
-  HIPCHK(h, hipMemsetAsync(rx.counters.p, 0, CT_COUNT * sizeof(uint64_t), h->stream));
+  if (int rcb = rx_block_counters(h)) return rcb;
+  HIPCHK(h, hipMemsetAsync(rx_ctr(h), 0, CT_COUNT * sizeof(uint64_t), h->stream));
   if (c.npeaks == 0) {
     HIPCHK(h, hipStreamSynchronize(h->stream));
     c.done = true;
@@ -729,7 +756,7 @@
   dq.smap = h->d_smap.as<int16_t>();
   dq.constellation = h->d_const.as<c32>();
   dq.grid = h->has_grid ? h->d_grid.as<SlicerGrid>() : nullptr;
-  dq.invalid = rx.invalid.as<uint8_t>();
+  dq.invalid = rx.rb_dev<uint8_t>(RB_INVALID);
   dq.res = rx.res.as<FrameResult>();
   dq.raw = rx.raw.as<uint8_t>();
   if (rx.quality_on) {
@@ -772,11 +799,10 @@
   const uint64_t nframes = c.nframes;
   HIPCHK(h, rx.res.ensure(nframes * sizeof(FrameResult)));
   HIPCHK(h, rx.raw.ensure(nframes * (uint64_t)RAW_SLOT));
-  HIPCHK(h, rx.invalid.ensure(nframes));
   HIPCHK(h, rx.chain_list.ensure(4096 * sizeof(uint32_t)));
   HIPCHK(h, rx.key.ensure(nframes * sizeof(uint64_t)));
   HIPCHK(h, rx.pos.ensure(nframes * sizeof(uint64_t)));
-  HIPCHK(h, hipMemsetAsync(rx.invalid.p, 0, nframes, h->stream));
+  HIPCHK(h, hipMemsetAsync(rx.rb_dev<uint8_t>(RB_INVALID), 0, nframes, h->stream));
   int rc = make_demod_params(c);
   if (rc) return rc;
   ProfScope span(h->prof, OFDM_K_DEMOD, h->stream);
@@ -804,7 +830,7 @@
   }
   hipLaunchKernelGGL(k_chain_resolve, dim3(1), dim3(64), 0, h->stream, rx.res.as<FrameResult>(), nframes, c.dynf,
                      rx.chain_list.as<uint32_t>(), 4096u, reinterpret_cast<const unsigned int*>(ctr + CT_CHAIN),
-                     rx.invalid.as<uint8_t>(), reinterpret_cast<unsigned int*>(ctr + CT_OVERFLOW), rx.pre_inv.as<uint8_t>(), npre);
+                     rx.rb_dev<uint8_t>(RB_INVALID), reinterpret_cast<unsigned int*>(ctr + CT_OVERFLOW), rx.pre_inv.as<uint8_t>(), npre);
   HIPCHK(h, hipGetLastError());
   if (npre) HIPCHK(h, hipStreamSynchronize(h->stream));
   return OFDM_OK;
@@ -868,7 +894,7 @@
   fq.dyn = c.dynf;
   fq.nframes = (uint32_t)c.nframes;
   fq.res = rx.res.as<FrameResult>();
-  fq.invalid = rx.invalid.as<uint8_t>();
+  fq.invalid = rx.rb_dev<uint8_t>(RB_INVALID);
   fq.raw = rx.raw.as<uint8_t>();
   fq.mask = h->d_mask.as<uint8_t>();
   fq.crc_table = h->d_crc.as<uint32_t>();
@@ -903,7 +929,7 @@
   QualityParams qw;
   qw.fq = rx.qual_frame.as<FrameQuality>();
   qw.step = rx.step.as<double>();
-  qw.out = rx.qual_out.as<ofdm_pkt_quality>();
+  qw.out = rx.rb_dev<ofdm_pkt_quality>(RB_QUAL_OUT);
   qw.inv_npilot = h->q_npilot ? 1.0f / (float)h->q_npilot : 0.0f;
   qw.inv_nnull = h->q_nnull ? 1.0f / (float)h->q_nnull : 0.0f;
   qw.N = h->N;
@@ -919,10 +945,6 @@
   const uint64_t npk_ub = c.npk_ub = c.dyn ? std::min<uint64_t>(nframes, (uint64_t)c.max_pkts) : c.npk;
   c.d_pay = c.payload_out;
   if (npk_ub == 0) return OFDM_OK;
-  HIPCHK(h, rx.out_off.ensure((npk_ub + 1) * sizeof(uint64_t)));
-  HIPCHK(h, rx.out_len.ensure(npk_ub * sizeof(uint32_t)));
-  HIPCHK(h, rx.out_ok.ensure(npk_ub));
-  HIPCHK(h, rx.out_pos.ensure(npk_ub * sizeof(uint64_t)));
   if (!h->dev_ptrs) {
     const uint64_t stage = c.dyn ? std::min<uint64_t>(c.payload_cap, nframes * (uint64_t)OFDM_MAX_PKT_LEN) : c.nbytes;
     HIPCHK(h, rx.out_payload.ensure(std::max<uint64_t>(stage, 1)));
@@ -930,17 +952,16 @@
   }
   fq.payload_out = c.d_pay;
   fq.payload_cap = c.dyn ? c.payload_cap : c.nbytes;
-  fq.out_off = rx.out_off.as<uint64_t>();
-  fq.out_len = rx.out_len.as<uint32_t>();
-  fq.out_ok = rx.out_ok.as<uint8_t>();
-  fq.out_pos = rx.out_pos.as<uint64_t>();
+  fq.out_off = rx.rb_dev<uint64_t>(RB_OUT_OFF);
+  fq.out_len = rx.rb_dev<uint32_t>(RB_OUT_LEN);
+  fq.out_ok = rx.rb_dev<uint8_t>(RB_OUT_OK);
+  fq.out_pos = rx.rb_dev<uint64_t>(RB_OUT_POS);
   fq.peaks = rx.peaks.as<uint64_t>();
   fq.j0 = (uint32_t)c.n_lo;
   fq.max_pkts = (uint32_t)npk_ub;
   hipLaunchKernelGGL(k_deframe_write, dim3((unsigned)((nframes + 3) / 4)), dim3(256), 0, h->stream, fq);
   HIPCHK(h, hipGetLastError());
   if (rx.quality_on) {
-    HIPCHK(h, rx.qual_out.ensure(npk_ub * sizeof(ofdm_pkt_quality)));
     hipLaunchKernelGGL(k_quality_write, dim3((unsigned)((nframes + 255) / 256)), dim3(256), 0, h->stream, fq, make_quality_params(h));
     HIPCHK(h, hipGetLastError());
   }
@@ -958,16 +979,6 @@
                        rx.raw_tap.as<uint8_t>());
     HIPCHK(h, hipGetLastError());
   }
-  HIPCHK(h, hipMemcpyAsync(c.payload_off, rx.out_off.p, npk_ub * sizeof(uint64_t), hipMemcpyDeviceToHost, h->stream));
-  HIPCHK(h, hipMemcpyAsync(c.payload_len, rx.out_len.p, npk_ub * sizeof(uint32_t), hipMemcpyDeviceToHost, h->stream));
-  HIPCHK(h, hipMemcpyAsync(c.crc_ok, rx.out_ok.p, npk_ub, hipMemcpyDeviceToHost, h->stream));
-  rx.last_pos.resize(npk_ub);
-  HIPCHK(h, hipMemcpyAsync(rx.last_pos.data(), rx.out_pos.p, npk_ub * sizeof(uint64_t), hipMemcpyDeviceToHost, h->stream));
-  if (rx.quality_on) {
-    rx.last_quality.resize(npk_ub);
-    HIPCHK(h, hipMemcpyAsync(rx.last_quality.data(), rx.qual_out.p, npk_ub * sizeof(ofdm_pkt_quality), hipMemcpyDeviceToHost,
-                             h->stream));
-  }
   if (!c.dyn && !h->dev_ptrs && c.nbytes)
     HIPCHK(h, hipMemcpyAsync(c.payload_out, c.d_pay, c.nbytes, hipMemcpyDeviceToHost, h->stream));
   return OFDM_OK;
@@ -976,30 +987,36 @@
 static int rx_finish(RxCall& c) {
   ofdm_handle* h = c.h;
   RxState& rx = h->rx;
-  int rc = rx_read_counts(c);
+  int rc = rx_read_counts(c, rx.rb_lay.total);
   if (rc) return rc;
   const uint64_t npk = c.npk, nframes = c.nframes;
+  rx.last_pos = rx.rb_mirror<uint64_t>(RB_OUT_POS);
+  rx.last_pos_n = std::min<uint64_t>(npk, c.npk_ub);
+  if (rx.quality_on) {
+    rx.last_quality = rx.rb_mirror<ofdm_pkt_quality>(RB_QUAL_OUT);
+    rx.last_quality_n = rx.last_pos_n;
+  }
   if (c.dyn) {
-    rx.last_pos.resize(std::min<uint64_t>(npk, c.npk_ub));
-    if (rx.quality_on) rx.last_quality.resize(std::min<uint64_t>(npk, c.npk_ub));
     if ((rc = rx_check_capacity(c))) return rc;
     if (!h->dev_ptrs && c.nbytes) HIPCHK(h, hipMemcpy(c.payload_out, c.d_pay, c.nbytes, hipMemcpyDeviceToHost));
   }
-  rx.last_swallowed.assign(rx.npeaks, 0);
-  if (nframes) {
-    std::vector<uint8_t> inv(nframes);
-    HIPCHK(h, hipMemcpy(inv.data(), rx.invalid.p, nframes, hipMemcpyDeviceToHost));
-    for (uint64_t f = 0; f < nframes && rx.j0 + f < rx.npeaks; f++) rx.last_swallowed[rx.j0 + f] = inv[f];
-  }
-  if (npk > 0) c.payload_off[npk] = c.nbytes;
+  rx.last_swallowed = rx.rb_mirror<uint8_t>(RB_INVALID);
+  rx.last_swallowed_n = nframes;
+  const uint8_t* ok = rx.rb_mirror<uint8_t>(RB_OUT_OK);
+  if (npk > 0) {
+    memcpy(c.payload_off, rx.rb_mirror<uint64_t>(RB_OUT_OFF), npk * sizeof(uint64_t));
+    memcpy(c.payload_len, rx.rb_mirror<uint32_t>(RB_OUT_LEN), npk * sizeof(uint32_t));
+    memcpy(c.crc_ok, ok, npk);
+    c.payload_off[npk] = c.nbytes;
+  }
   *c.npkt = (int)npk;
   if (rx.csi_on) {
     rx.csi_n = npk;
-    rx.csi_ok.assign(c.crc_ok, c.crc_ok + npk);
+    rx.csi_ok = ok;
   }
   if (c.stats) {
     uint64_t nok = 0;
-    for (uint64_t i = 0; i < npk; i++) nok += c.crc_ok[i] ? 1 : 0;
+    for (uint64_t i = 0; i < npk; i++) nok += ok[i] ? 1 : 0;
     c.stats->packets = npk;
     c.stats->crc_ok = nok;
   }
@@ -1016,13 +1033,9 @@
   RxState& rx = h->rx;
   rx.nsamples = c.nsamples;
   rx.npeaks = rx.nframes = rx.j0 = rx.nsym_total = rx.raw_tap_bytes = rx.run_slots = 0;
-  rx.last_pos.clear();
-  rx.last_swallowed.clear();
-  rx.last_quality.clear();
+  rx.drop_views();
   rx.quality_valid = rx.quality_on;
   rx.csi_valid = rx.csi_on;
-  rx.csi_n = 0;
-  rx.csi_ok.clear();
   if (c.stats) c.stats->samples = c.nsamples;
   return OFDM_OK;
 }
@@ -1066,7 +1079,9 @@
   if ((rc = rx_timing(c)) || c.done) return rc;
   c.dyn = rx_counts_on_device(h);
   c.nframes = c.npeaks;
-  if (!c.dyn && ((rc = rx_read_counts(c)) || c.nframes == 0)) return rc;
+  if (!c.dyn && ((rc = rx_read_counts(c, CT_COUNT * sizeof(uint64_t))) || c.nframes == 0)) return rc;
+  if ((rc = rx_block_fit(h, rx_readback_layout(std::min<uint64_t>(c.nframes, (uint64_t)c.max_pkts), c.nframes, h->rx.quality_on))))
+    return rc;
   c.dynf.lo = c.dyn ? reinterpret_cast<const unsigned int*>(rx_ctr(h) + CT_NLO) : nullptr;
   c.dynf.hi = c.dyn ? reinterpret_cast<const unsigned int*>(rx_ctr(h) + CT_NHI) : nullptr;
   c.dynf.npeaks = (uint32_t)c.npeaks;
@@ -1074,7 +1089,7 @@
   {
     ProfScope span(h->prof, OFDM_K_DEFRAME, h->stream);
     if ((rc = rx_chains(c)) || (rc = rx_tap_pass(c)) || (rc = rx_deframe_count(c))) return rc;
-    if (!c.dyn && ((rc = rx_read_counts(c)) || (rc = rx_check_capacity(c)))) return rc;
+    if (!c.dyn && ((rc = rx_read_counts(c, CT_COUNT * sizeof(uint64_t))) || (rc = rx_check_capacity(c)))) return rc;
     if ((rc = rx_outputs(c))) return rc;
   }
   return rx_finish(c);
@@ -1241,11 +1256,11 @@
 
 extern "C" int ofdm_rx_packet_pos(ofdm_handle* h, uint64_t* pos, int cap, int* n) {
   if (!h) return OFDM_E_INVAL;
-  const size_t np = h->rx.last_pos.size();
+  const size_t np = (size_t)h->rx.last_pos_n;
   if (n) *n = (int)np;
   if (np == 0 || !pos) return OFDM_OK;
   if ((size_t)cap < np) FAIL(h, OFDM_E_CAPACITY, "position array too small");
-  memcpy(pos, h->rx.last_pos.data(), np * sizeof(uint64_t));
+  memcpy(pos, h->rx.last_pos, np * sizeof(uint64_t));
   return OFDM_OK;
 }
 
@@ -1256,7 +1271,9 @@
   if (n) *n = (int)std::min<uint64_t>(rx.npeaks, 0x7FFFFFFF);
   if (rx.npeaks == 0 || (!peaks && !phi && !step && !swallowed)) return OFDM_OK;
   if (!peaks || !phi || !step || !swallowed || (uint64_t)cap < rx.npeaks) FAIL(h, OFDM_E_CAPACITY, "NCO state arrays too small");
-  for (uint64_t i = 0; i < rx.npeaks; i++) swallowed[i] = i < rx.last_swallowed.size() ? rx.last_swallowed[i] : 0;
+  memset(swallowed, 0, rx.npeaks);
+  if (rx.last_swallowed && rx.j0 < rx.npeaks)
+    memcpy(swallowed + rx.j0, rx.last_swallowed, std::min<uint64_t>(rx.last_swallowed_n, rx.npeaks - rx.j0));
   HIPCHK(h, hipSetDevice(h->cfg.device_id));
   HIPCHK(h, hipMemcpy(peaks, rx.peaks.p, rx.npeaks * sizeof(uint64_t), hipMemcpyDeviceToHost));
   HIPCHK(h, hipMemcpy(phi, rx.Phi_u.p, rx.npeaks * sizeof(uint64_t), hipMemcpyDeviceToHost));
@@ -1280,11 +1297,11 @@
   if (!h) return OFDM_E_INVAL;
   const RxState& rx = h->rx;
   if (!rx.quality_valid) FAIL(h, OFDM_E_INVAL, "the last ofdm_rx ran without link quality (ofdm_set_rx_quality)");
-  const size_t np = rx.last_quality.size();
+  const size_t np = (size_t)rx.last_quality_n;
   if (n) *n = (int)np;
   if (np == 0 || !out) return OFDM_OK;
   if ((size_t)cap < np) FAIL(h, OFDM_E_CAPACITY, "quality array too small");
-  memcpy(out, rx.last_quality.data(), np * sizeof(ofdm_pkt_quality));
+  memcpy(out, rx.last_quality, np * sizeof(ofdm_pkt_quality));
   return OFDM_OK;
 }
 
@@ -1339,7 +1356,7 @@
   HIPCHK(h, hipSetDevice(h->cfg.device_id));
   CsiSumParams s;
   s.rows = csi_packet_rows(rx);
-  s.ok = rx.out_ok.as<uint8_t>();
+  s.ok = rx.rb_dev<uint8_t>(RB_OUT_OK);
   s.npk = (uint32_t)rx.csi_n;
   s.occ = occ;
   s.stride = rx.csi_stride;
diff --git a/ofdm_uhd_amd/csrc/rx_readback.h b/ofdm_uhd_amd/csrc/rx_readback.h
--- /dev/null
+++ b/ofdm_uhd_amd/csrc/rx_readback.h
@@ -0,0 +1,50 @@
+#pragma once
+#include <stddef.h>
+#include <stdint.h>
+
+#include "../../include/ofdm_hip.h"
+
+enum { CT_CAND = 0, CT_OVERFLOW = 1, CT_NLO = 2, CT_NHI = 3, CT_CHAIN = 4, CT_NPEAKS = 5, CT_NSYM = 6, CT_KEYTOT = 7,
+       CT_DEFR = 8 , CT_RAWTOT = 13, CT_PIECES = 14, CT_STASH = 15, CT_RECS = 16, CT_COUNT = 17 };
+
+enum {
+  RB_COUNTERS = 0,
+  RB_INVALID,
+  RB_OUT_POS,
+  RB_OUT_OFF,
+  RB_OUT_LEN,
+  RB_OUT_OK,
+  RB_QUAL_OUT,
+  RB_NSECT
+};
+
+struct RbSection {
+  size_t off, bytes;
+};
+struct RxReadback {
+  RbSection s[RB_NSECT];
+  size_t total;
+};
+
+#define RB_ALIGN 16
+
+static inline RxReadback rx_readback_layout(uint64_t npk_ub, uint64_t nframes, bool quality_on) {
+  const size_t bytes[RB_NSECT] = {
+      CT_COUNT * sizeof(uint64_t),
+      (size_t)nframes,
+      (size_t)npk_ub * sizeof(uint64_t),
+      npk_ub ? ((size_t)npk_ub + 1) * sizeof(uint64_t) : 0,
+      (size_t)npk_ub * sizeof(uint32_t),
+      (size_t)npk_ub,
+      quality_on ? (size_t)npk_ub * sizeof(ofdm_pkt_quality) : 0,
+  };
+  RxReadback lay;
+  size_t at = 0;
+  for (int k = 0; k < RB_NSECT; k++) {
+    lay.s[k].off = at;
+    lay.s[k].bytes = bytes[k];
+    at = (at + bytes[k] + (RB_ALIGN - 1)) & ~(size_t)(RB_ALIGN - 1);
+  }
+  lay.total = at;
+  return lay;
+}
diff --git a/ofdm_uhd_amd/csrc/rx_state.h b/ofdm_uhd_amd/csrc/rx_state.h
--- a/ofdm_uhd_amd/csrc/rx_state.h
+++ b/ofdm_uhd_amd/csrc/rx_state.h
@@ -1,14 +1,14 @@
 #pragma once
 #include "host_util.h"
 #include "rx_demod.h"
+#include "rx_readback.h"
 
 #define RX_DEVBUFS(X)                                                                                                       \
   X(recs) X(x_stage) X(y) X(metric) X(presel) X(tile_B) X(tile_np) X(tile_first) X(tile_pieces) X(avg_in) X(cand_u)        \
-  X(cand_P) X(counters) X(counts) X(offsets) X(partial) X(peaks) X(peak_P) X(angle) X(step) X(inc) X(Phi) X(K) X(nsym)     \
-  X(sym_base) X(res) X(raw) X(invalid) X(chain_list) X(key) X(pos) X(out_payload) X(out_off) X(out_len) X(out_ok)          \
-  X(out_pos) X(inc_acc) X(Phi_u) X(peaks2) X(peak_P2) X(fstep) X(pre_inv) X(stash_peaks) X(stash_P) X(tap_fft) X(tap_acq)  \
-  X(tap_sink) X(tap_demapped) X(raw_tap) X(raw_lens) X(raw_pos) X(tap_sampler) X(tap_sigmix) X(tap_nco) X(qual_frame)      \
-  X(qual_out) X(csi_frame) X(csi_rows) X(csi_part) X(csi_sum) X(run_rows)
+  X(cand_P) X(rb) X(counts) X(offsets) X(partial) X(peaks) X(peak_P) X(angle) X(step) X(inc) X(Phi) X(K) X(nsym)           \
+  X(sym_base) X(res) X(raw) X(chain_list) X(key) X(pos) X(out_payload) X(inc_acc) X(Phi_u) X(peaks2) X(peak_P2) X(fstep)   \
+  X(pre_inv) X(stash_peaks) X(stash_P) X(tap_fft) X(tap_acq) X(tap_sink) X(tap_demapped) X(raw_tap) X(raw_lens) X(raw_pos) \
+  X(tap_sampler) X(tap_sigmix) X(tap_nco) X(qual_frame) X(csi_frame) X(csi_rows) X(csi_part) X(csi_sum) X(run_rows)
 
 struct RxState {
 #define X(name) DevBuf name;
@@ -24,7 +24,18 @@
   uint64_t sub_n = 0;
   const c32* sub_dx = nullptr;
   uint64_t origin = 0;
-  std::vector<uint64_t> last_pos;
+  PinBuf rb_host;
+  RxReadback rb_lay = rx_readback_layout(0, 0, false);
+  template <typename T>
+  T* rb_dev(int sect) const {
+    return reinterpret_cast<T*>(static_cast<uint8_t*>(rb.p) + rb_lay.s[sect].off);
+  }
+  template <typename T>
+  const T* rb_mirror(int sect) const {
+    return reinterpret_cast<const T*>(static_cast<const uint8_t*>(rb_host.p) + rb_lay.s[sect].off);
+  }
+  const uint64_t* last_pos = nullptr;
+  uint64_t last_pos_n = 0;
   bool nco_ref_on = false;
   int64_t nco_ref_peak = 0, nco_trust_after = 0;
   uint64_t nco_ref_u = 0;
@@ -32,14 +43,25 @@
   std::vector<uint64_t> hist_flags;
   std::vector<double> hist_steps;
   std::vector<uint8_t> hist_swallowed;
-  std::vector<uint8_t> last_swallowed;
+  const uint8_t* last_swallowed = nullptr;
+  uint64_t last_swallowed_n = 0;
   bool quality_on = false, quality_valid = false;
-  std::vector<ofdm_pkt_quality> last_quality;
+  const ofdm_pkt_quality* last_quality = nullptr;
+  uint64_t last_quality_n = 0;
   bool csi_on = false, csi_valid = false;
   uint64_t csi_n = 0, csi_rows_cap = 0;
   int csi_stride = 0;
-  std::vector<uint8_t> csi_ok;
+  const uint8_t* csi_ok = nullptr;
+  void drop_views() {
+    last_pos = nullptr;
+    last_swallowed = nullptr;
+    last_quality = nullptr;
+    csi_ok = nullptr;
+    last_pos_n = last_swallowed_n = last_quality_n = csi_n = 0;
+  }
   void release() {
+    rb_host.release();
+    drop_views();
 #define X(name) name.release();
     RX_DEVBUFS(X)
 #undef X
```

New measurement: 132.3 million OFDM symbols/s. Within noise of the previous version (-0.0%).
